# jwliao1209/DiffMusic

Hardware: AMD Instinct MI355X
Metric: denoising steps/sec (10 s clip, 200-step DPS) (higher is better)
Workload: dtype f16; 1 GPU; MusicLDM + DPS music_inpainting, 10 s @16 kHz, 200-step schedule, batch 8 per GPU (BASELINE.json configs[1]); global_batch=8, clips_per_gpu=8, lanes=1, parallelism=clip-sharded x1 (RCCL world size 1, no per-step collective), finite=True, nan_steps=0, settle_steps=10, cached_reference_transform=True, launched_by=single process

## Files before the change

### diffmusic_amd/_lib.py

```python
import ctypes as C
import os

_HERE = os.path.dirname(os.path.abspath(__file__))
LIB_PATH = os.environ.get("DMX_LIB_PATH") or os.path.join(_HERE, "lib", "libdiffmusic_hip.so")
MAX_STAGES = 8


class HifiGanConfig(C.Structure):
    _fields_ = [("model_in_dim", C.c_int), ("upsample_initial_channel", C.c_int), ("num_upsamples", C.c_int),
                ("upsample_rates", C.c_int * MAX_STAGES), ("upsample_kernel_sizes", C.c_int * MAX_STAGES),
                ("num_kernels", C.c_int), ("resblock_kernel_sizes", C.c_int * MAX_STAGES),
                ("num_dilations", C.c_int), ("resblock_dilation_sizes", C.c_int * (MAX_STAGES * MAX_STAGES)),
                ("leaky_relu_slope", C.c_float)]


class VaeConfig(C.Structure):
    _fields_ = [("latent_channels", C.c_int), ("out_channels", C.c_int), ("num_blocks", C.c_int),
                ("block_out_channels", C.c_int * MAX_STAGES), ("layers_per_block", C.c_int),
                ("norm_num_groups", C.c_int), ("eps", C.c_float)]


class UNetConfig(C.Structure):
    _fields_ = [("in_channels", C.c_int), ("out_channels", C.c_int), ("num_blocks", C.c_int),
                ("block_out_channels", C.c_int * MAX_STAGES), ("layers_per_block", C.c_int),
# ... 1 lines not shown
                ("down_attn", C.c_int * MAX_STAGES), ("up_attn", C.c_int * MAX_STAGES),
                ("class_embed_dim", C.c_int), ("num_attn_per_layer", C.c_int), ("attn_cross_dims", C.c_int * 4)]


class HtsatConfig(C.Structure):
    _fields_ = [("spec_size", C.c_int), ("num_mel_bins", C.c_int), ("patch_size", C.c_int), ("embed_dim", C.c_int), ("window_size", C.c_int),
                ("num_stages", C.c_int), ("depths", C.c_int * 4), ("num_heads", C.c_int * 4), ("ln_eps", C.c_float), ("bn_eps", C.c_float)]


class GemmDesc(C.Structure):
    _fields_ = [("A", C.c_void_p), ("W", C.c_void_p), ("C", C.c_void_p), ("C2", C.c_void_p),
                ("bias", C.c_void_p), ("rowbias", C.c_void_p), ("R", C.c_void_p), ("X", C.c_void_p),
                ("M", C.c_int), ("N", C.c_int), ("K", C.c_int), ("ldw", C.c_int),
                ("Hi", C.c_int), ("Wi", C.c_int), ("Ci", C.c_int), ("lda", C.c_int),
                ("Hq", C.c_int), ("Wq", C.c_int), ("sy", C.c_int), ("sx", C.c_int),
                ("ntaps", C.c_int),
                ("Ho", C.c_int), ("Wo", C.c_int), ("ldc", C.c_int), ("osy", C.c_int), ("ooy", C.c_int),
                ("osx", C.c_int), ("oox", C.c_int),
                ("ldr", C.c_int), ("ldx", C.c_int), ("ldc2", C.c_int),
                ("Z", C.c_int), ("Zi", C.c_int),
                ("sAo", C.c_longlong), ("sAi", C.c_longlong), ("sWo", C.c_longlong), ("sWi", C.c_longlong),
                ("sCo", C.c_longlong), ("sCi", C.c_longlong),
                ("alpha", C.c_float), ("act_slope", C.c_float), ("mask_slope", C.c_float),
                ("flags", C.c_int),
                ("tdy", C.c_byte * 16), ("tdx", C.c_byte * 16), ("resid_inv_slope", C.c_float), ("tile_cfg", C.c_int), ("ldrb", C.c_int), ("ksplit", C.c_int),
                ("XB", C.c_void_p), ("B2", C.c_void_p), ("ldxb", C.c_int), ("ldb2", C.c_int),
                ("colsum", C.c_void_p), ("ln_eps", C.c_float), ("rowstats_in", C.c_void_p), ("rowstats_out", C.c_void_p), ("nslots", C.c_int),
                ("gn_part", C.c_void_p), ("gnb_x", C.c_void_p), ("gnb_scale", C.c_void_p), ("gnb_shift", C.c_void_p),
                ("gnb_ldx", C.c_int), ("gnb_silu", C.c_int), ("gnb_stats", C.c_void_p), ("gnb_cpg", C.c_int)]


EPI_BIAS, EPI_ROWBIAS, EPI_RESID, EPI_ACCUM, EPI_MASK, EPI_LRELU2, EPI_TANH, EPI_F32OUT, EPI_NO_C, EPI_RESID_INV, EPI_MASKBITS, EPI_BITS2, EPI_SOFTBWD = \
    1, 2, 4, 8, 16, 32, 64, 128, 256, 512, 1024, 2048, 4096
EPI_GEGLU, EPI_LNFOLD, EPI_ROWSTATS, EPI_GNSTATS, EPI_GNBWD = 8192, 16384, 32768, 65536, 131072

_SIGS = {
    "dmx_abi_version": (C.c_int, []),
    "dmx_act_dtype": (C.c_int, []),
    "dmx_last_error": (C.c_char_p, []),
    "dmx_hifigan_create": (C.c_void_p, [C.POINTER(HifiGanConfig)]),
    "dmx_vae_decoder_create": (C.c_void_p, [C.POINTER(VaeConfig)]),
    "dmx_unet_create": (C.c_void_p, [C.POINTER(UNetConfig)]),
    "dmx_model_destroy": (None, [C.c_void_p]),
    "dmx_model_num_params": (C.c_int, [C.c_void_p]),
    "dmx_model_param_name": (C.c_char_p, [C.c_void_p, C.c_int]),
    "dmx_model_param_numel": (C.c_size_t, [C.c_void_p, C.c_int]),
    "dmx_model_param_ndim": (C.c_int, [C.c_void_p, C.c_int]),
    "dmx_model_param_dim": (C.c_int, [C.c_void_p, C.c_int, C.c_int]),
    "dmx_model_load_param": (C.c_int, [C.c_void_p, C.c_char_p, C.c_void_p, C.c_size_t]),
    "dmx_model_finalize": (C.c_int, [C.c_void_p, C.c_void_p]),
    "dmx_hifigan_out_len": (C.c_int, [C.c_void_p, C.c_int]),
    "dmx_hifigan_workspace_bytes": (C.c_size_t, [C.c_void_p, C.c_int, C.c_int]),
    "dmx_hifigan_fwd": (C.c_int, [C.c_void_p, C.c_void_p, C.c_void_p, C.c_int, C.c_int, C.c_void_p, C.c_size_t, C.c_void_p]),
    "dmx_hifigan_bwd": (C.c_int, [C.c_void_p, C.c_void_p, C.c_void_p, C.c_void_p]),
    "dmx_hifigan_fwd_dead": (C.c_int, [C.c_void_p, C.c_void_p, C.c_void_p, C.c_int, C.c_int, C.c_int, C.c_int, C.c_void_p, C.c_size_t,
                                       C.c_void_p]),
    "dmx_hifigan_dead_plan": (C.c_int, [C.c_void_p, C.POINTER(C.c_int), C.POINTER(C.c_int), C.POINTER(C.c_int), C.POINTER(C.c_int), C.c_int]),
    "dmx_conv_dead_rows": (C.c_int, [C.c_int] * 9 + [C.POINTER(C.c_int), C.POINTER(C.c_int)]),
    "dmx_vae_workspace_bytes": (C.c_size_t, [C.c_void_p, C.c_int, C.c_int, C.c_int]),
    "dmx_vae_decode_fwd": (C.c_int, [C.c_void_p, C.c_void_p, C.c_float, C.c_void_p, C.c_void_p, C.c_int, C.c_int, C.c_int,
                                     C.c_int, C.c_void_p, C.c_size_t, C.c_void_p]),
    "dmx_vae_decode_bwd": (C.c_int, [C.c_void_p, C.c_void_p, C.c_float, C.c_void_p, C.c_void_p]),
    "dmx_vae_encoder_create": (C.c_void_p, [C.POINTER(VaeConfig)]),
    "dmx_vae_encoder_workspace_bytes": (C.c_size_t, [C.c_void_p, C.c_int, C.c_int, C.c_int]),
    "dmx_vae_encode_fwd": (C.c_int, [C.c_void_p, C.c_void_p, C.c_float, C.c_void_p, C.c_int, C.c_int, C.c_int, C.c_void_p, C.c_size_t,
                                     C.c_void_p]),
    "dmx_latent_init": (C.c_int, [C.c_void_p] * 6 + [C.c_int] * 3 + [C.c_float] * 3 + [C.c_void_p]),
    "dmx_conv2d_raw": (C.c_int, [C.c_void_p] * 4 + [C.c_int] * 9 + [C.c_void_p]),
    "dmx_unet_workspace_bytes": (C.c_size_t, [C.c_void_p, C.c_int, C.c_int, C.c_int]),
    "dmx_unet_fwd": (C.c_int, [C.c_void_p, C.c_void_p, C.c_void_p, C.c_void_p, C.c_void_p, C.c_int, C.c_int, C.c_int,
                               C.c_void_p, C.c_size_t, C.c_void_p]),
    "dmx_unet_fwd_ctx": (C.c_int, [C.c_void_p] * 5 + [C.c_int, C.c_void_p, C.c_int, C.c_void_p, C.c_void_p, C.c_int, C.c_int, C.c_int,
                                   C.c_void_p, C.c_size_t, C.c_void_p]),
    "dmx_unet_workspace_bytes_ctx": (C.c_size_t, [C.c_void_p, C.c_int, C.c_int, C.c_int, C.c_int, C.c_int]),
    "dmx_htsat_create": (C.c_void_p, [C.POINTER(HtsatConfig)]),
    "dmx_htsat_feature_dims": (C.c_int, [C.c_void_p, C.POINTER(C.c_int), C.POINTER(C.c_int)]),
    "dmx_htsat_workspace_bytes": (C.c_size_t, [C.c_void_p, C.c_int, C.c_int]),
    "dmx_htsat_fwd": (C.c_int, [C.c_void_p, C.c_void_p, C.c_int, C.c_int, C.c_void_p, C.c_int, C.c_void_p, C.c_size_t, C.c_void_p]),
    "dmx_htsat_bwd": (C.c_int, [C.c_void_p, C.c_void_p, C.c_void_p, C.c_void_p, C.c_void_p]),
    "dmx_htsat_tape_raw": (C.c_size_t, [C.c_void_p, C.c_int, C.c_int, C.c_int, C.c_void_p, C.c_size_t, C.c_void_p]),
    "dmx_gram_fwd": (C.c_int, [C.c_void_p, C.c_void_p, C.c_int, C.c_int, C.c_int, C.c_void_p]),
    "dmx_gram_bwd": (C.c_int, [C.c_void_p, C.c_void_p, C.c_void_p, C.c_int, C.c_int, C.c_int, C.c_void_p]),
    "dmx_gemm_raw": (C.c_int, [C.c_void_p, C.c_size_t, C.c_void_p]),
    "dmx_prof_begin": (None, []),
    "dmx_prof_end": (C.c_int, [C.POINTER(C.c_double), C.POINTER(C.c_double)]),
    "dmx_flash_attn_raw": (C.c_int, [C.c_void_p, C.c_void_p, C.c_void_p, C.c_void_p, C.c_void_p] + [C.c_int] * 6 + [C.c_float, C.c_void_p]),
    "dmx_flash_attn_ld_raw": (C.c_int, [C.c_void_p] * 5 + [C.c_int] * 8 + [C.c_float, C.POINTER(C.c_int), C.c_void_p]),
    "dmx_softmax_raw": (C.c_int, [C.c_void_p] * 3 + [C.c_longlong, C.c_int, C.c_longlong, C.c_longlong, C.c_int, C.c_void_p]),
    "dmx_softmax_act_raw": (C.c_int, [C.c_void_p] * 3 + [C.c_longlong, C.c_int, C.c_longlong, C.c_int, C.c_void_p]),
    "dmx_transpose_raw": (C.c_int, [C.c_void_p, C.c_void_p, C.c_int, C.c_int, C.c_longlong, C.c_longlong, C.c_int, C.c_int] + [C.c_longlong] * 4
                          + [C.c_void_p]),
    "dmx_rowdot_raw": (C.c_int, [C.c_void_p] * 3 + [C.c_longlong, C.c_int, C.c_longlong, C.c_longlong, C.c_void_p]),
    "dmx_layernorm_raw": (C.c_int, [C.c_void_p] * 4 + [C.c_int, C.c_int, C.c_float, C.c_void_p]),
    "dmx_geglu_raw": (C.c_int, [C.c_void_p, C.c_void_p, C.c_longlong, C.c_int, C.c_void_p]),
    "dmx_gemm_splitk_workspace": (C.c_int, [C.c_void_p, C.c_size_t]),
    "dmx_conv_pair_raw": (C.c_int, [C.c_void_p, C.c_void_p, C.c_size_t, C.c_void_p]),
    "dmx_conv_pair_group_raw": (C.c_int, [C.c_int, C.c_void_p, C.c_void_p, C.c_size_t, C.c_void_p]),
    "dmx_conv_pair_dead_raw": (C.c_int, [C.c_void_p, C.c_void_p, C.c_size_t, C.POINTER(C.c_int), C.POINTER(C.c_int), C.POINTER(C.c_int), C.c_void_p]),
    "dmx_conv_pair_group_dead_raw": (C.c_int, [C.c_int, C.c_void_p, C.c_void_p, C.c_size_t, C.POINTER(C.c_int), C.c_void_p]),
    "dmx_groupnorm_scratch_floats": (C.c_size_t, [C.c_int, C.c_int, C.c_int]),
    "dmx_groupnorm_raw": (C.c_int, [C.c_void_p] * 8 + [C.c_int] * 4 + [C.c_float, C.c_int, C.c_void_p]),
    "dmx_groupnorm_part_floats": (C.c_size_t, [C.c_int, C.c_int, C.c_int]),
    "dmx_groupnorm_parts_raw": (C.c_int, [C.c_void_p] * 7 + [C.c_int] * 4 + [C.c_float, C.c_int, C.c_int, C.c_void_p, C.c_void_p, C.c_void_p]),
    "dmx_gemm_last_tile_rows_raw": (C.c_int, []),
    "dmx_groupnorm_bwd_raw": (C.c_int, [C.c_void_p] * 10 + [C.c_int] * 6 + [C.c_void_p, C.c_void_p, C.c_void_p]),
    "dmx_prof_dominant": (C.c_int, [C.POINTER(C.c_double)] * 3),
    "dmx_audio_create": (C.c_void_p, [C.c_int, C.c_int, C.c_int, C.c_int, C.c_void_p]),
    "dmx_audio_destroy": (None, [C.c_void_p]),
    "dmx_audio_num_frames": (C.c_int, [C.c_void_p, C.c_int]),
    "dmx_audio_num_bins": (C.c_int, [C.c_void_p]),
    "dmx_audio_state_bytes": (C.c_size_t, [C.c_void_p, C.c_int, C.c_int]),
    "dmx_audio_transform_fwd": (C.c_int, [C.c_void_p, C.c_void_p, C.c_longlong, C.c_void_p, C.c_void_p, C.c_int, C.c_int, C.c_int,
                                          C.c_int, C.c_float, C.c_float, C.c_void_p]),
    "dmx_audio_transform_bwd": (C.c_int, [C.c_void_p, C.c_void_p, C.c_void_p, C.c_longlong, C.c_void_p, C.c_int, C.c_int, C.c_int,
                                          C.c_int, C.c_float, C.c_float, C.c_int, C.c_void_p]),
    "dmx_audio_is_fused": (C.c_int, [C.c_void_p, C.c_int]),
    "dmx_audio_guidance_fwd": (C.c_int, [C.c_void_p, C.c_void_p, C.c_longlong, C.c_void_p, C.c_void_p, C.c_longlong, C.c_void_p, C.c_void_p,
                                         C.c_int, C.c_int, C.c_int, C.c_int, C.c_float, C.c_float, C.c_void_p]),
    "dmx_audio_guidance_bwd": (C.c_int, [C.c_void_p, C.c_void_p, C.c_longlong, C.c_void_p, C.c_void_p, C.c_longlong, C.c_float, C.c_void_p,
                                         C.c_void_p, C.c_longlong, C.c_int, C.c_void_p, C.c_int, C.c_int, C.c_int, C.c_int, C.c_float, C.c_float,
                                         C.c_void_p]),
    "dmx_audio_guidance_fwd_ex": (C.c_int, [C.c_void_p, C.c_void_p, C.c_longlong, C.c_void_p, C.c_void_p, C.c_longlong, C.c_void_p, C.c_void_p,
                                            C.c_int, C.c_int, C.c_int, C.c_int, C.c_float, C.c_float, C.c_void_p, C.c_longlong, C.c_void_p,
                                            C.c_float, C.c_void_p]),
    "dmx_audio_guidance_bwd_ex": (C.c_int, [C.c_void_p, C.c_void_p, C.c_longlong, C.c_void_p, C.c_void_p, C.c_longlong, C.c_float, C.c_void_p,
                                            C.c_void_p, C.c_longlong, C.c_int, C.c_void_p, C.c_int, C.c_int, C.c_int, C.c_int, C.c_float, C.c_float,
                                            C.c_void_p, C.c_longlong, C.c_void_p, C.c_float, C.c_void_p]),
    "dmx_audio_guidance_fwd_shaped": (C.c_int, [C.c_void_p, C.c_void_p, C.c_longlong, C.c_void_p, C.c_void_p, C.c_longlong, C.c_void_p, C.c_void_p,
                                                C.c_int, C.c_int, C.c_int, C.c_int, C.c_float, C.c_float, C.c_void_p, C.c_longlong, C.c_void_p,
                                                C.c_float, C.c_void_p, C.c_void_p]),
    "dmx_audio_guidance_bwd_shaped": (C.c_int, [C.c_void_p, C.c_void_p, C.c_longlong, C.c_void_p, C.c_void_p, C.c_longlong, C.c_float, C.c_void_p,
                                                C.c_void_p, C.c_longlong, C.c_int, C.c_void_p, C.c_int, C.c_int, C.c_int, C.c_int, C.c_float, C.c_float,
                                                C.c_void_p, C.c_longlong, C.c_void_p, C.c_float, C.c_void_p, C.c_void_p]),
    "dmx_clip_fwd": (C.c_int, [C.c_void_p, C.c_longlong, C.c_void_p, C.c_void_p, C.c_longlong, C.c_int, C.c_int, C.c_void_p]),
    "dmx_clip_bwd": (C.c_int, [C.c_void_p, C.c_longlong, C.c_void_p, C.c_longlong, C.c_void_p, C.c_void_p, C.c_longlong, C.c_int, C.c_int, C.c_int,
                               C.c_void_p]),
    "dmx_declip_project": (C.c_int, [C.c_void_p, C.c_longlong, C.c_void_p, C.c_longlong, C.c_void_p, C.c_void_p, C.c_longlong, C.c_int, C.c_int,
                                     C.c_void_p]),
    "dmx_drc_fwd": (C.c_int, [C.c_void_p, C.c_longlong, C.c_void_p, C.c_longlong, C.c_void_p, C.c_void_p, C.c_int, C.c_int] + [C.c_float] * 6 +
                    [C.c_void_p]),
    "dmx_drc_bwd": (C.c_int, [C.c_void_p, C.c_longlong, C.c_void_p, C.c_longlong, C.c_void_p, C.c_void_p, C.c_void_p, C.c_void_p, C.c_longlong,
                              C.c_int, C.c_int, C.c_int] + [C.c_float] * 6 + [C.c_void_p]),
    "dmx_drc_fwd_p": (C.c_int, [C.c_void_p, C.c_longlong, C.c_void_p, C.c_longlong, C.c_void_p, C.c_void_p, C.c_void_p, C.c_int, C.c_int, C.c_float,
                                C.c_void_p]),
    "dmx_drc_bwd_p": (C.c_int, [C.c_void_p, C.c_longlong, C.c_void_p, C.c_longlong] + [C.c_void_p] * 6 + [C.c_longlong, C.c_int, C.c_int, C.c_int,
                                                                                                        C.c_float, C.c_void_p]),
    "dmx_drc_pgrad": (C.c_int, [C.c_void_p] * 6 + [C.c_int, C.c_int, C.c_float, C.c_void_p]),
    "dmx_drc_update": (C.c_int, [C.c_void_p] * 5 + [C.c_int] * 3 + [C.c_void_p] + [C.c_double] * 3 + [C.c_float, C.c_void_p, C.c_void_p, C.c_void_p]),
    "dmx_warp_fwd": (C.c_int, [C.c_void_p, C.c_longlong, C.c_void_p, C.c_longlong, C.c_void_p, C.c_int, C.c_int, C.c_void_p]),
    "dmx_warp_bwd": (C.c_int, [C.c_void_p, C.c_void_p, C.c_longlong, C.c_void_p, C.c_int, C.c_int, C.c_int, C.c_void_p]),
    "dmx_warp_wgrad": (C.c_int, [C.c_void_p, C.c_void_p, C.c_longlong, C.c_void_p, C.c_longlong, C.c_void_p, C.c_int, C.c_int, C.c_void_p]),
    "dmx_warp_update": (C.c_int, [C.c_void_p] * 5 + [C.c_int] * 4 + [C.c_double] * 5 + [C.c_int, C.c_void_p]),
    "dmx_click_detect": (C.c_int, [C.c_void_p, C.c_longlong] + [C.c_void_p] * 5 + [C.c_int, C.c_int, C.c_float, C.c_float, C.c_void_p]),
    "dmx_click_mask": (C.c_int, [C.c_void_p, C.c_void_p, C.c_void_p, C.c_int, C.c_int, C.c_int, C.c_void_p]),
    "dmx_mask_rows": (C.c_int, [C.c_void_p, C.c_longlong, C.c_void_p, C.c_longlong, C.c_void_p, C.c_int, C.c_int, C.c_int, C.c_void_p]),
    "dmx_declick_blend": (C.c_int, [C.c_void_p, C.c_longlong, C.c_void_p, C.c_longlong, C.c_void_p, C.c_longlong, C.c_void_p, C.c_int, C.c_int,
                                    C.c_int, C.c_void_p]),
    "dmx_noise_add": (C.c_int, [C.c_void_p, C.c_void_p, C.c_void_p, C.c_longlong, C.c_float, C.c_void_p]),
    "dmx_audio_stft_mag": (C.c_int, [C.c_void_p, C.c_void_p, C.c_longlong, C.c_void_p, C.c_void_p, C.c_int, C.c_int, C.c_void_p]),
    "dmx_audio_stft_mag_bwd": (C.c_int, [C.c_void_p, C.c_void_p, C.c_void_p, C.c_longlong, C.c_void_p, C.c_int, C.c_int, C.c_int, C.c_void_p]),
    "dmx_audio_tf_frames": (C.c_int, [C.c_int]),
    "dmx_audio_tf_gain": (C.c_int, [C.c_void_p, C.c_void_p, C.c_longlong, C.c_void_p, C.c_longlong, C.c_void_p, C.c_longlong, C.c_int, C.c_int, C.c_int,
                                    C.c_void_p]),
    "dmx_audio_tf_curve": (C.c_int, [C.c_void_p, C.c_void_p, C.c_longlong, C.c_void_p, C.c_longlong, C.c_void_p, C.c_longlong, C.c_int, C.c_int, C.c_int,
                                     C.c_void_p]),
    "dmx_audio_tf_wgrad_segments": (C.c_int, [C.c_int]),
    "dmx_audio_tf_wgrad": (C.c_int, [C.c_void_p, C.c_void_p, C.c_longlong, C.c_void_p, C.c_longlong, C.c_void_p, C.c_int, C.c_int, C.c_void_p]),
    "dmx_audio_eq_update": (C.c_int, [C.c_void_p, C.c_int] + [C.c_void_p] * 3 + [C.c_int, C.c_int] + [C.c_double] * 4 + [C.c_int, C.c_void_p]),
    "dmx_audio_melscale": (C.c_int, [C.c_void_p, C.c_void_p, C.c_void_p, C.c_int, C.c_int, C.c_float, C.c_float, C.c_void_p]),
    "dmx_mask_apply": (C.c_int, [C.c_void_p, C.c_longlong, C.c_void_p, C.c_void_p, C.c_longlong, C.c_int, C.c_int, C.c_int, C.c_void_p]),
    "dmx_l2_loss": (C.c_int, [C.c_void_p, C.c_longlong, C.c_void_p, C.c_void_p, C.c_void_p, C.c_int, C.c_longlong, C.c_float, C.c_void_p]),
    "dmx_track_stitch_fwd": (C.c_int, [C.c_void_p, C.c_longlong, C.c_void_p, C.POINTER(C.c_int)] + [C.c_int] * 4 + [C.c_void_p]),
    "dmx_track_stitch_bwd": (C.c_int, [C.c_void_p, C.c_void_p, C.c_longlong, C.POINTER(C.c_int)] + [C.c_int] * 5 + [C.c_void_p]),
    "dmx_stem_mix_fwd": (C.c_int, [C.c_void_p, C.c_longlong, C.c_void_p, C.POINTER(C.c_float)] + [C.c_int] * 3 + [C.c_void_p]),
    "dmx_stem_mix_bwd": (C.c_int, [C.c_void_p, C.c_void_p, C.c_longlong, C.POINTER(C.c_float)] + [C.c_int] * 4 + [C.c_void_p]),
    "dmx_stem_project": (C.c_int, [C.c_void_p, C.c_longlong, C.c_void_p, C.c_void_p, C.POINTER(C.c_float), C.c_int, C.c_int, C.c_void_p]),
    "dmx_grad_normalize": (C.c_int, [C.c_void_p, C.c_void_p, C.c_int, C.c_longlong, C.c_float, C.c_void_p]),
    "dmx_fir_fwd": (C.c_int, [C.c_void_p, C.c_longlong, C.c_void_p, C.c_void_p, C.c_longlong] + [C.c_int] * 7 + [C.c_void_p]),
    "dmx_fir_bwd": (C.c_int, [C.c_void_p, C.c_longlong, C.c_void_p, C.c_void_p, C.c_void_p, C.c_longlong] + [C.c_int] * 7 + [C.c_void_p]),
    "dmx_fir_clip_fwd": (C.c_int, [C.c_void_p, C.c_longlong, C.c_void_p, C.c_void_p, C.c_longlong] + [C.c_int] * 4 + [C.c_void_p]),
    "dmx_fir_clip_bwd": (C.c_int, [C.c_void_p, C.c_longlong, C.c_void_p, C.c_void_p, C.c_void_p, C.c_longlong] + [C.c_int] * 4 + [C.c_void_p]),
    "dmx_fir_wgrad_workspace_floats": (C.c_size_t, [C.c_int, C.c_int, C.c_int]),
    "dmx_fir_wgrad": (C.c_int, [C.c_void_p, C.c_longlong, C.c_void_p, C.c_longlong, C.c_void_p, C.c_size_t] + [C.c_int] * 4 + [C.c_void_p]),
    "dmx_ir_update": (C.c_int, [C.c_void_p, C.c_int] + [C.c_void_p] * 4 + [C.c_int, C.c_int] + [C.c_double] * 4 + [C.c_int, C.c_void_p]),
    "dmx_sched_pred_x0": (C.c_int, [C.c_void_p, C.c_void_p, C.c_void_p, C.c_longlong, C.c_float, C.c_void_p]),
    "dmx_sched_pred_x0_ex": (C.c_int, [C.c_void_p, C.c_void_p, C.c_void_p, C.c_longlong, C.c_float, C.c_int, C.c_float, C.c_void_p]),
    "dmx_sched_step_ex": (C.c_int, [C.c_int] + [C.c_void_p] * 9 + [C.c_int, C.c_int] + [C.c_float] * 5 + [C.c_int, C.c_int, C.c_float, C.c_void_p]),
    "dmx_sched_cfg_combine": (C.c_int, [C.c_void_p, C.c_void_p, C.c_longlong, C.c_float, C.c_void_p]),
    "dmx_randn_philox": (C.c_int, [C.c_void_p, C.c_int, C.c_longlong, C.POINTER(C.c_ulonglong), C.c_ulonglong, C.c_void_p]),
    "dmx_sched_step": (C.c_int, [C.c_int] + [C.c_void_p] * 9 + [C.c_int, C.c_int] + [C.c_float] * 5 + [C.c_int, C.c_void_p]),
}

ADDED_IN_V4 = ("dmx_vae_encoder_create", "dmx_vae_encoder_workspace_bytes", "dmx_vae_encode_fwd", "dmx_latent_init",
               "dmx_track_stitch_fwd", "dmx_track_stitch_bwd", "dmx_audio_guidance_fwd_shaped", "dmx_audio_guidance_bwd_shaped",
               "dmx_clip_fwd", "dmx_clip_bwd", "dmx_declip_project", "dmx_hifigan_fwd_dead", "dmx_hifigan_dead_plan", "dmx_conv_dead_rows",
               "dmx_fir_clip_fwd", "dmx_fir_clip_bwd", "dmx_fir_wgrad", "dmx_fir_wgrad_workspace_floats", "dmx_ir_update",
               "dmx_stem_mix_fwd", "dmx_stem_mix_bwd", "dmx_stem_project", "dmx_audio_tf_gain", "dmx_audio_tf_frames",
               "dmx_audio_tf_curve", "dmx_audio_tf_wgrad_segments", "dmx_audio_tf_wgrad", "dmx_audio_eq_update", "dmx_drc_fwd", "dmx_drc_bwd",
               "dmx_warp_fwd", "dmx_warp_bwd", "dmx_warp_wgrad", "dmx_warp_update", "dmx_drc_fwd_p", "dmx_drc_bwd_p", "dmx_drc_pgrad",
               "dmx_drc_update", "dmx_click_detect", "dmx_click_mask", "dmx_mask_rows", "dmx_declick_blend")

_lib = None


def check_symbols(h, path=LIB_PATH):
    for name in ADDED_IN_V4:
        if not hasattr(h, name):
            raise RuntimeError(f"{path} reports ABI version {ABI_VERSION} but does not export `{name}` (a build from before the VAE "
                               "encoder / track-mode / declipping / blind-dereverberation / source-separation / time-frequency-masking / blind-equalisation / de-compression / wow-and-flutter / blind-wow-and-flutter / blind-de-compression / declicking entry points): rebuild it (python -m diffmusic_amd.build --force)")


def lib():
    global _lib
    if _lib is None:
        if not os.path.exists(LIB_PATH):
            raise RuntimeError(f"{LIB_PATH} is missing: build it with `python -m diffmusic_amd.build` "
                               "(the diffmusic_amd hot path has no CPU fallback)")
        h = C.CDLL(LIB_PATH)
        for name, (res, args) in _SIGS.items():
            if not hasattr(h, name):
                continue
            fn = getattr(h, name)
            fn.restype, fn.argtypes = res, args
        if h.dmx_abi_version() != ABI_VERSION:
            raise RuntimeError(f"libdiffmusic_hip.so ABI version {h.dmx_abi_version()} != {ABI_VERSION} expected by this package: rebuild it "
                               "(python -m diffmusic_amd.build --force)")
        check_symbols(h)
        _lib = h
    return _lib


ABI_VERSION = 4


def act_dtype():
    import torch
    return torch.float16 if lib().dmx_act_dtype() == 1 else torch.bfloat16


class DmxError(RuntimeError):
    pass


def check(rc, what=""):
    if rc != 0:
        msg = lib().dmx_last_error()
        raise DmxError(f"{what} failed with code {rc}: {msg.decode() if msg else ''}")
```

### diffmusic_amd/csrc/capi.hip

```cpp
#include "conv_pair.h"
#include "models.h"

#define M_IMPL(m) ((m) ? (m)->impl : nullptr)
#define ST(s) ((hipStream_t)(s))

extern "C" {

int dmx_abi_version(void) { return DMX_ABI_VERSION; }
int dmx_act_dtype(void) { return DMX_ACT_DTYPE; }

dmx_model* dmx_hifigan_create(const dmx_hifigan_config* cfg) {
  if (!cfg || cfg->num_upsamples > DMX_MAX_STAGES || cfg->num_kernels > DMX_MAX_STAGES || cfg->num_dilations > DMX_MAX_STAGES) {
    dmx_set_error("bad hifigan config");
    return nullptr;
  }
  return new dmx_model{dmx_make_hifigan(cfg)};
}
dmx_model* dmx_vae_decoder_create(const dmx_vae_config* cfg) {
  if (!cfg || cfg->num_blocks > DMX_MAX_STAGES) { dmx_set_error("bad vae config"); return nullptr; }
  Model* m = dmx_make_vae(cfg);
  return m ? new dmx_model{m} : nullptr;
}
dmx_model* dmx_unet_create(const dmx_unet_config* cfg) {
  if (!cfg || cfg->num_blocks > DMX_MAX_STAGES) { dmx_set_error("bad unet config"); return nullptr; }
// ... 81 lines not shown
  return dmx_vae_enc_ws_impl(m->impl, batch, frames, bins);
}
int dmx_vae_encode_fwd(dmx_model* m, const float* mel, float log_floor, float* moments, int batch, int frames, int bins, void* ws,
                       size_t ws_bytes, void* stream) {
  int rc = check(m, DMX_MODEL_VAE_ENC);
  if (rc) return rc;
  if (!ws) { dmx_set_error("null workspace"); return DMX_ERR_WORKSPACE; }
  return dmx_vae_enc_fwd_impl(m->impl, mel, log_floor, moments, batch, frames, bins, ws, ws_bytes, ST(stream));
}
int dmx_latent_init(const float* moments, float* mean, float* logvar, float* x, const float* eps, const float* noise, int batch,
                    int latent_channels, int hw, float sqrt_abar, float scaling_factor, float sqrt_1m_abar, void* stream) {
  return dmx_latent_init_impl(moments, mean, logvar, x, eps, noise, batch, latent_channels, hw, sqrt_abar, scaling_factor, sqrt_1m_abar, ST(stream));
}
int dmx_conv2d_raw(const float* w_host, const float* b_host, const void* x, void* y, int B, int Hi, int Wi, int Ci, int Co, int k, int stride,
                   int pad_lo, int pad_hi, void* stream) {
  return dmx_conv2d_raw_impl(w_host, b_host, (const act_t*)x, (act_t*)y, B, Hi, Wi, Ci, Co, k, stride, pad_lo, pad_hi, ST(stream));
}

dmx_model* dmx_htsat_create(const dmx_htsat_config* cfg) {
  Model* impl = dmx_make_htsat(cfg);
  if (!impl) return nullptr;
  return new dmx_model{impl};
}
int dmx_htsat_feature_dims(dmx_model* m, int* tokens, int* channels) {
  if (!m || !m->impl || m->impl->kind != DMX_MODEL_HTSAT) { dmx_set_error("wrong model handle"); return DMX_ERR_STATE; }
  dmx_htsat_dims_impl(m->impl, tokens, channels);
  return DMX_OK;
}
size_t dmx_htsat_workspace_bytes(dmx_model* m, int batch, int frames) {
  if (!m || !m->impl || m->impl->kind != DMX_MODEL_HTSAT) return 0;
  return dmx_htsat_ws_impl(m->impl, batch, frames);
}
int dmx_htsat_fwd(dmx_model* m, const float* mel, int batch, int frames, float* feat, int keep_state, void* ws, size_t ws_bytes, void* stream) {
  int rc = check(m, DMX_MODEL_HTSAT);
  if (rc) return rc;
  if (!ws) { dmx_set_error("null workspace"); return DMX_ERR_WORKSPACE; }
  return dmx_htsat_fwd_impl(m->impl, mel, batch, frames, feat, keep_state, ws, ws_bytes, ST(stream));
}
int dmx_htsat_bwd(dmx_model* m, const float* dfeat, const float* scale, float* dmel, void* stream) {
  int rc = check(m, DMX_MODEL_HTSAT);
  if (rc) return rc;
  return dmx_htsat_bwd_impl(m->impl, dfeat, scale, dmel, ST(stream));
}
size_t dmx_htsat_tape_raw(dmx_model* m, int stage, int block, int which, void* dst, size_t dst_elems, void* stream) {
  if (!m || !m->impl || m->impl->kind != DMX_MODEL_HTSAT) return 0;
  const act_t* p = nullptr;
  const size_t n = dmx_htsat_tape_impl(m->impl, stage, block, which, &p);
  if (n && dst && dst_elems >= n) (void)hipMemcpyAsync(dst, p, n * sizeof(act_t), hipMemcpyDeviceToDevice, ST(stream));
  return n;
}
int dmx_gram_fwd(const float* F, float* G, int batch, int tokens, int channels, void* stream) {
  const int rc = dmx_gram_fwd_impl(F, G, batch, tokens, channels, ST(stream));
  if (rc == DMX_ERR_SHAPE) dmx_set_error("gram: 1 <= tokens <= 96");
  return rc;
}
int dmx_gram_bwd(const float* F, const float* dG, float* dF, int batch, int tokens, int channels, void* stream) {
  return dmx_gram_bwd_impl(F, dG, dF, batch, tokens, channels, ST(stream));
}

size_t dmx_unet_workspace_bytes(dmx_model* m, int batch, int h, int w) { return dmx_unet_ws_impl(m->impl, batch, h, w, 0, 0); }
size_t dmx_unet_workspace_bytes_ctx(dmx_model* m, int batch, int h, int w, int n0, int n1) { return dmx_unet_ws_impl(m->impl, batch, h, w, n0, n1); }
int dmx_unet_fwd(dmx_model* m, const float* x, const float* t, const float* class_labels, float* eps, int batch, int h, int w,
                 void* ws, size_t ws_bytes, void* stream) {
  int rc = check(m, DMX_MODEL_UNET);
  if (rc) return rc;
  if (!ws) { dmx_set_error("null workspace"); return DMX_ERR_WORKSPACE; }
  return dmx_unet_fwd_impl(m->impl, x, t, class_labels, eps, batch, h, w, ws, ws_bytes, ST(stream), nullptr, 0, nullptr, 0, nullptr);
}
int dmx_unet_fwd_ctx(dmx_model* m, const float* x, const float* t, const float* class_labels, const float* ctx0, int n0,
                     const float* ctx1, int n1, const float* bias1, float* eps, int batch, int h, int w, void* ws, size_t ws_bytes,
                     void* stream) {
  int rc = check(m, DMX_MODEL_UNET);
  if (rc) return rc;
  if (!ws) { dmx_set_error("null workspace"); return DMX_ERR_WORKSPACE; }
  return dmx_unet_fwd_impl(m->impl, x, t, class_labels, eps, batch, h, w, ws, ws_bytes, ST(stream), ctx0, n0, ctx1, n1, bias1);
}

static thread_local int g_raw_gn_rows = 0;
int dmx_gemm_raw(const void* desc, size_t desc_bytes, void* stream) {
  if (desc_bytes != sizeof(GemmDesc)) { dmx_set_error("GemmDesc size mismatch: %zu vs %zu", desc_bytes, sizeof(GemmDesc)); return DMX_ERR_SHAPE; }
  return dmx_gemm_launch(*reinterpret_cast<const GemmDesc*>(desc), ST(stream), &g_raw_gn_rows);
}
int dmx_gemm_last_tile_rows_raw(void) { return g_raw_gn_rows; }

int dmx_conv_pair_raw(const void* desc_a, const void* desc_b, size_t desc_bytes, void* stream) {
  if (desc_bytes != sizeof(GemmDesc)) { dmx_set_error("GemmDesc size mismatch: %zu vs %zu", desc_bytes, sizeof(GemmDesc)); return DMX_ERR_SHAPE; }
  const GemmDesc* a = reinterpret_cast<const GemmDesc*>(desc_a);
  const GemmDesc& b = *reinterpret_cast<const GemmDesc*>(desc_b);
  if (!dmx_conv_pair_eligible(a, b)) { dmx_set_error("shape not handled by the fused convolution-pair kernel"); return DMX_ERR_SHAPE; }
  return dmx_conv_pair_launch(a, b, ST(stream));
}

int dmx_conv_pair_group_raw(int n, const void* descs_a, const void* descs_b, size_t desc_bytes, void* stream) {
  if (desc_bytes != sizeof(GemmDesc)) { dmx_set_error("GemmDesc size mismatch: %zu vs %zu", desc_bytes, sizeof(GemmDesc)); return DMX_ERR_SHAPE; }
  if (n < 1 || n > 3) { dmx_set_error("conv pair group: 1..3 problems"); return DMX_ERR_SHAPE; }
  const GemmDesc* a = reinterpret_cast<const GemmDesc*>(descs_a);
  const GemmDesc* b = reinterpret_cast<const GemmDesc*>(descs_b);
  const GemmDesc* pa[3]; const GemmDesc* pb[3];
  for (int j = 0; j < n; ++j) { pa[j] = a + j; pb[j] = b + j; }
  const int rc = dmx_conv_pair_group_launch(n, pa, pb, ST(stream));
  if (rc == DMX_ERR_SHAPE) dmx_set_error("shape not handled by the fused convolution-pair kernel");
  return rc;
}

static PairDead pair_dead_of(const int* d) { PairDead pd; pd.skip0 = d[0]; pd.skip1 = d[1]; pd.zero0 = d[2]; pd.zero1 = d[3]; return pd; }

int dmx_conv_pair_dead_raw(const void* desc_a, const void* desc_b, size_t desc_bytes, const int* dead, int* skipped, int* total, void* stream) {
  if (skipped) *skipped = 0;
  if (total) *total = 0;
  if (desc_bytes != sizeof(GemmDesc)) { dmx_set_error("GemmDesc size mismatch: %zu vs %zu", desc_bytes, sizeof(GemmDesc)); return DMX_ERR_SHAPE; }
  const GemmDesc* a = reinterpret_cast<const GemmDesc*>(desc_a);
  const GemmDesc& b = *reinterpret_cast<const GemmDesc*>(desc_b);
  if (!dmx_conv_pair_eligible(a, b)) { dmx_set_error("shape not handled by the fused convolution-pair kernel"); return DMX_ERR_SHAPE; }
  PairDead pd;
  if (dead) pd = pair_dead_of(dead);
  int sk = 0, tot = 0;
  dmx_conv_pair_slabs(a, b, dead ? &pd : nullptr, &sk, &tot);
  if (skipped) *skipped = sk;
  if (total) *total = tot;
  const int rc = dmx_conv_pair_launch(a, b, ST(stream), dead ? &pd : nullptr);
  if (rc == DMX_ERR_SHAPE) dmx_set_error("dead rows not handled by the fused convolution-pair kernel (zero rows need the residual to be stage a's input)");
  return rc;
}

int dmx_conv_pair_group_dead_raw(int n, const void* descs_a, const void* descs_b, size_t desc_bytes, const int* dead, void* stream) {
  if (desc_bytes != sizeof(GemmDesc)) { dmx_set_error("GemmDesc size mismatch: %zu vs %zu", desc_bytes, sizeof(GemmDesc)); return DMX_ERR_SHAPE; }
  if (n < 1 || n > 3) { dmx_set_error("conv pair group: 1..3 problems"); return DMX_ERR_SHAPE; }
  const GemmDesc* a = reinterpret_cast<const GemmDesc*>(descs_a);
  const GemmDesc* b = reinterpret_cast<const GemmDesc*>(descs_b);
  const GemmDesc* pa[3]; const GemmDesc* pb[3];
  PairDead pd[3];
  for (int j = 0; j < n; ++j) { pa[j] = a + j; pb[j] = b + j; if (dead) pd[j] = pair_dead_of(dead + 4 * j); }
  const int rc = dmx_conv_pair_group_launch(n, pa, pb, ST(stream), dead ? pd : nullptr);
  if (rc == DMX_ERR_SHAPE) dmx_set_error("shape not handled by the fused convolution-pair kernel");
  return rc;
}

int dmx_flash_attn_raw(const void* q, const void* k, const void* v, void* o, const float* colbias, int B, int Nq, int Nk, int ldv, int C,
                       int heads, float scale, void* stream) {
  const int rc = dmx_flash_attn_fwd((const act_t*)q, (const act_t*)k, (const act_t*)v, (act_t*)o, colbias, B, Nq, Nk, C, heads, scale,
                                    ST(stream), 0, 0, ldv);
  if (rc == DMX_ERR_SHAPE) dmx_set_error("flash attention: unsupported head_dim / strides");
  return rc;
}

int dmx_flash_attn_ld_raw(const void* q, const void* k, const void* v, void* o, const float* colbias, int B, int Nq, int Nk, int ldq, int ldk,
                          int ldv, int C, int heads, float scale, int* qt_out, void* stream) {
  if (qt_out) *qt_out = 0;
  if (B < 1 || heads < 1 || C < heads || C % heads) { dmx_set_error("flash attention: C %d is not heads %d x head_dim", C, heads); return DMX_ERR_SHAPE; }
  const int rc = dmx_flash_attn_fwd((const act_t*)q, (const act_t*)k, (const act_t*)v, (act_t*)o, colbias, B, Nq, Nk, C, heads, scale,
                                    ST(stream), ldq, ldk, ldv, qt_out);
  if (rc == DMX_ERR_SHAPE)
    dmx_set_error("flash attention: head_dim %d (multiples of 8 up to 96), Nq %d, Nk %d (>= 1) or row strides %d / %d / %d (multiples of 8) unsupported",
                  C / heads, Nq, Nk, ldq, ldk, ldv);
  return rc;
}

int dmx_softmax_raw(const float* S, void* P, const float* colbias, long long rows, int N, long long lds, long long ldp, int rows_per_bias,
                    void* stream) {
  const int rc = dmx_softmax_fwd(S, (act_t*)P, colbias, rows, N, lds, ldp, rows_per_bias, ST(stream));
  if (rc == DMX_ERR_SHAPE) dmx_set_error("softmax: N %d (a multiple of 4, <= 4096), lds %lld, ldp %lld (multiples of 4) unsupported", N, lds, ldp);
  return rc;
}
int dmx_softmax_act_raw(const void* S, void* P, const float* colbias, long long rows, int N, long long ldp, int rows_per_bias, void* stream) {
  const int rc = dmx_softmax_act((const act_t*)S, (act_t*)P, colbias, rows, N, ldp, rows_per_bias, ST(stream));
  if (rc == DMX_ERR_SHAPE) dmx_set_error("softmax: N %d (a multiple of 4, <= 4096), ldp %lld (a multiple of 4) unsupported", N, ldp);
// ... 75 lines not shown
```

### diffmusic_amd/csrc/dmx_common.h

```cpp
#pragma once
#include <hip/hip_runtime.h>
#include <stdint.h>
#include <stddef.h>

typedef uint16_t act_t;

#define DMX_OK 0
#define DMX_ERR_SHAPE (-1)
#define DMX_ERR_WORKSPACE (-2)
#define DMX_ERR_PARAM (-3)
#define DMX_ERR_STATE (-4)
#define DMX_ERR_LAUNCH (-5)

typedef __attribute__((ext_vector_type(4))) float f32x4;
#ifdef DMX_BF16
typedef __bf16 native16_t;
typedef __attribute__((ext_vector_type(8))) __bf16 frag8_t;
#define DMX_MFMA16(a, b, c) __builtin_amdgcn_mfma_f32_16x16x32_bf16(a, b, c, 0, 0, 0)
#define DMX_ACT_DTYPE 0
#else
typedef _Float16 native16_t;
typedef __attribute__((ext_vector_type(8))) _Float16 frag8_t;
#define DMX_MFMA16(a, b, c) __builtin_amdgcn_mfma_f32_16x16x32_f16(a, b, c, 0, 0, 0)
#define DMX_ACT_DTYPE 1
// ... 33 lines not shown
  float r = 0.f;
  for (int i = 0; i < nw; ++i) r += sh[i];
  return r;
}
__device__ __forceinline__ float block_max(float v, float* sh) {
  v = wave_max(v);
  const int w = threadIdx.x >> 6, nw = blockDim.x >> 6;
  __syncthreads();
  if ((threadIdx.x & 63) == 0) sh[w] = v;
  __syncthreads();
  float r = -3.0e38f;
  for (int i = 0; i < nw; ++i) r = fmaxf(r, sh[i]);
  return r;
}

static inline int cdiv(int a, int b) { return (a + b - 1) / b; }
static inline size_t align_up(size_t v, size_t a) { return (v + a - 1) / a * a; }

#define DMX_MAX_TAPS 16
enum {
  EPI_BIAS = 1,
  EPI_ROWBIAS = 2,
  EPI_RESID = 4,
  EPI_ACCUM = 8,
  EPI_MASK = 16,
  EPI_LRELU2 = 32,
  EPI_TANH = 64,
  EPI_F32OUT = 128,
  EPI_NO_C = 256,
  EPI_RESID_INV = 512,
  EPI_MASKBITS = 1024,
  EPI_BITS2 = 2048,
  EPI_GEGLU = 8192,
  EPI_LNFOLD = 16384,
  EPI_ROWSTATS = 32768,
  EPI_GNSTATS = 65536,
  EPI_GNBWD = 131072,
  EPI_BIASINIT = 262144,
  EPI_SOFTBWD = 4096
};

struct GemmDesc {
  const act_t* A;
  const act_t* W;
  void* C;
  act_t* C2;
  const float* bias;
  const float* rowbias;
  const act_t* R;
  const act_t* X;
  int M, N, K;
  int ldw;
  int Hi, Wi, Ci, lda;
  int Hq, Wq, sy, sx;
  int ntaps;
  int Ho, Wo, ldc, osy, ooy, osx, oox;
  int ldr, ldx, ldc2;
  int Z, Zi;
  long long sAo, sAi, sWo, sWi, sCo, sCi;
  float alpha, act_slope, mask_slope;
  int flags;
  signed char tdy[DMX_MAX_TAPS], tdx[DMX_MAX_TAPS];
  float resid_inv_slope;
  int tile_cfg;
  int ldrb;
  int ksplit;
  const unsigned char* XB;
  unsigned char* B2;
  int ldxb, ldb2;
  const float* colsum;
  float ln_eps;
  const float* rowstats_in;
  float* rowstats_out;
  int nslots;
  float* gn_part;
  const act_t* gnb_x;
  const float* gnb_scale;
  const float* gnb_shift;
  int gnb_ldx, gnb_silu;
  const float* gnb_stats;
  int gnb_cpg;
};

int dmx_gemm_launch(const GemmDesc& d, hipStream_t stream, int* gn_rows = nullptr);
void dmx_gemm_set_splitk_workspace(float* ws, size_t bytes);
void dmx_gemm_release_splitk_workspace(const float* ws);
int dmx_gemm_launch_ln(int cfg, const GemmDesc& d, hipStream_t stream);
int dmx_gemm_launch_rowstats(int cfg, const GemmDesc& d, hipStream_t stream);
int dmx_gemm_launch_gnstats(int cfg, const GemmDesc& d, hipStream_t stream, int* gn_rows);
bool dmx_prof_is_active();
```

### diffmusic_amd/csrc/gemm_conv.hip

```cpp
#include "gemm_tile.h"

namespace {
template <int BM, int BN, int WM, int WN, int NSTAGE>
int launch_glds(const GemmDesc& d, hipStream_t stream) {
  if (d.flags & EPI_SOFTBWD) {
    if constexpr (BM == 256 && BN == 256) return launch_glds_t<BM, BN, WM, WN, NSTAGE, 2>(d, stream);
    else return DMX_ERR_SHAPE;
  }
  if (d.flags & EPI_GEGLU) return launch_glds_t<BM, BN, WM, WN, NSTAGE, 3>(d, stream);
  return (d.flags & (EPI_MASKBITS | EPI_BITS2)) ? launch_glds_t<BM, BN, WM, WN, NSTAGE, 1>(d, stream)
                                                : launch_glds_t<BM, BN, WM, WN, NSTAGE, 0>(d, stream);
}

template <int BM, int BN, int WM, int WN>
int launch_cfg(const GemmDesc& d, hipStream_t stream) {
  if (d.flags & EPI_SOFTBWD) return DMX_ERR_SHAPE;
  if (d.flags & EPI_GEGLU) {
    if constexpr ((BN / WN) % 32 == 0) return launch_cfg_t<BM, BN, WM, WN, 3>(d, stream);
    else return DMX_ERR_SHAPE;
  }
  return (d.flags & (EPI_MASKBITS | EPI_BITS2)) ? launch_cfg_t<BM, BN, WM, WN, 1>(d, stream) : launch_cfg_t<BM, BN, WM, WN, 0>(d, stream);
}

}
// ... 180 lines not shown
  }
  if (flags & EPI_RESID) {
    const uint2 rr = *reinterpret_cast<const uint2*>(p.R + row * p.ldr + n);
    const float is = (flags & EPI_RESID_INV) ? p.resid_inv_slope : 1.f;
    const float x[4] = {alo(rr.x), ahi(rr.x), alo(rr.y), ahi(rr.y)};
#pragma unroll
    for (int e = 0; e < 4; ++e) a[e] += fminf(x[e], x[e] * is);
  }
#pragma unroll
  for (int e = 0; e < 4; ++e) a[e] *= p.alpha;
  if (!(flags & EPI_NO_C))
    *reinterpret_cast<uint2*>(reinterpret_cast<act_t*>(p.C) + row * p.ldc + n) = make_uint2(pack2a(a[0], a[1]), pack2a(a[2], a[3]));
  if (flags & EPI_LRELU2) {
    const float sl = p.act_slope;
    *reinterpret_cast<uint2*>(p.C2 + row * p.ldc2 + n) =
        make_uint2(pack2a(fmaxf(a[0], a[0] * sl), fmaxf(a[1], a[1] * sl)), pack2a(fmaxf(a[2], a[2] * sl), fmaxf(a[3], a[3] * sl)));
  }
}

int splitk_plan(const GemmDesc& d, int* tile) {
  static const bool off = getenv("DMX_NO_SPLITK") != nullptr;
  if (off || !g_splitk_ws || d.Z != 1 || !glds_ok(d)) return 1;
  if (d.flags & (EPI_ACCUM | EPI_F32OUT | EPI_TANH | EPI_MASKBITS | EPI_BITS2 | EPI_SOFTBWD | EPI_GEGLU | EPI_LNFOLD | EPI_ROWSTATS)) return 1;
  if (!(d.osy == 1 && d.osx == 1 && d.ooy == 0 && d.oox == 0 && d.Ho == d.Hq && d.Wo == d.Wq)) return 1;
  if ((d.N & 7) || (d.ldc & 3)) return 1;
  const int nk = (d.K + BK - 1) / BK;
  auto fits = [&](int ks) { return ks >= 2 && ks <= nk && (size_t)ks * d.M * d.N * sizeof(float) <= g_splitk_bytes; };
  auto dma_tile = [](int t) { return t == 1 || t == 2 || (t >= 7 && t <= 19); };
  if (d.tile_cfg >= 100) { *tile = d.tile_cfg % 100; return fits(d.tile_cfg / 100) && dma_tile(*tile) ? d.tile_cfg / 100 : 1; }
  if (d.tile_cfg) return 1;
  for (const TileEntry* e = g_tile_table; e->cfg; ++e)
    if (e->M == d.M && e->N == d.N && e->K == d.K && e->Z == d.Z) {
      if (e->cfg < 100) return 1;
      *tile = e->cfg % 100;
      return fits(e->cfg / 100) && dma_tile(*tile) ? e->cfg / 100 : 1;
    }
  if (d.M > 8192) return 1;
  const long long tiles = (long long)cdiv(d.M, 64) * cdiv(d.N, 64);
  if (nk < 24 || tiles >= 256) return 1;
  int ks = (int)(1024 / tiles);
  if (ks > nk / 8) ks = nk / 8;
  if (ks > 8) ks = 8;
  while (ks > 1 && !fits(ks)) --ks;
  *tile = d.N % 128 == 0 && d.M >= 4096 ? 14 : 12;
  return ks < 2 ? 1 : ks;
}

int launch_splitk(const GemmDesc& d, int ks, int tile, hipStream_t stream) {
  GemmDesc g = d;
  g.ksplit = ks;
  g.flags = EPI_F32OUT;
  g.C = g_splitk_ws; g.C2 = nullptr; g.ldc = d.N; g.alpha = 1.f;
  g.bias = nullptr; g.rowbias = nullptr; g.R = nullptr; g.X = nullptr;
  g.Ho = d.Hq; g.Wo = d.Wq;
  g.tile_cfg = 0;
  int rc = launch_by_cfg(tile, g, stream);
  if (rc != DMX_OK) return rc;
  const long long nthr = (long long)d.M * (d.N >> 2);
  hipLaunchKernelGGL(splitk_epilogue_kernel, dim3((unsigned)((nthr + 255) / 256)), dim3(256), 0, stream, d, g_splitk_ws, ks);
  g_last_cfg = 100 * ks + tile;
  return hipGetLastError() == hipSuccess ? DMX_OK : DMX_ERR_LAUNCH;
}
}

void dmx_gemm_set_splitk_workspace(float* ws, size_t bytes) { g_splitk_ws = ws; g_splitk_bytes = bytes; }
void dmx_gemm_release_splitk_workspace(const float* ws) { if (g_splitk_ws == ws) { g_splitk_ws = nullptr; g_splitk_bytes = 0; } }

int dmx_prof_open(hipStream_t st) {
  if (!g_prof) return -1;
  ProfRec r;
  memset(&r, 0, sizeof(r));
  (void)hipEventCreate(&r.a); (void)hipEventCreate(&r.b);
  (void)hipEventRecord(r.a, st);
  g_prof_recs.push_back(r);
  return (int)g_prof_recs.size() - 1;
}
void dmx_prof_close(int rec, hipStream_t st, double flops, double bytes, int M, int N, int K, int taps, int flags, int cfg) {
  if (rec < 0 || rec >= (int)g_prof_recs.size()) return;
  ProfRec& r = g_prof_recs[rec];
  (void)hipEventRecord(r.b, st);
  r.flops = flops; r.bytes = bytes; r.M = M; r.N = N; r.K = K; r.Z = 1; r.taps = taps; r.flags = flags; r.cfg = cfg;
}

int dmx_gemm_launch(const GemmDesc& d, hipStream_t stream, int* gn_rows) {
  if (gn_rows) *gn_rows = 0;
  if (d.M <= 0 || d.N <= 0 || d.K <= 0) return DMX_ERR_SHAPE;
  if ((d.Ci & 7) || (d.N & 3) || (d.K & 7) || (d.lda & 7) || (d.ldw & 7) || (d.ldc & 3)) return DMX_ERR_SHAPE;
  if (d.ntaps < 1 || d.ntaps > DMX_MAX_TAPS || d.K != d.ntaps * d.Ci) return DMX_ERR_SHAPE;
  if (d.Z < 1 || d.Zi < 1) return DMX_ERR_SHAPE;
  if ((d.flags & EPI_LRELU2) && !(d.act_slope >= 0.f && d.act_slope <= 1.f)) return DMX_ERR_SHAPE;
  if ((d.flags & EPI_RESID_INV) && !(d.resid_inv_slope >= 1.f)) return DMX_ERR_SHAPE;
  if (d.flags & EPI_SOFTBWD) {
    if ((d.flags & ~(EPI_SOFTBWD)) || ((d.N | d.ldc | d.ldx) & 7) || !d.X || !d.rowbias || d.Zi != 1 || d.ntaps != 1) return DMX_ERR_SHAPE;
    if (!(d.osy == 1 && d.osx == 1 && d.ooy == 0 && d.oox == 0 && d.Ho == d.Hq && d.Wo == d.Wq)) return DMX_ERR_SHAPE;
  }
  if (d.flags & EPI_GEGLU) {
    if ((d.flags & ~(EPI_GEGLU | EPI_BIAS | EPI_LNFOLD)) || (d.N & 31) || (d.ldc & 7) || d.ldc < d.N / 2 || d.alpha != 1.f) return DMX_ERR_SHAPE;
    if ((d.ldr | d.ldx | d.ldc2) & 7) return DMX_ERR_SHAPE;
    if (!(d.osy == 1 && d.osx == 1 && d.ooy == 0 && d.oox == 0 && d.Ho == d.Hq && d.Wo == d.Wq)) return DMX_ERR_SHAPE;
  }
  if (d.flags & (EPI_MASKBITS | EPI_BITS2)) {
    if ((d.flags & EPI_F32OUT) || ((d.N | d.ldc | d.ldr | d.ldx | d.ldc2) & 7) || d.Z != 1) return DMX_ERR_SHAPE;
    if ((d.flags & EPI_MASKBITS) && (!d.XB || d.ldxb * 8 < d.N)) return DMX_ERR_SHAPE;
    if ((d.flags & EPI_BITS2) && (!d.B2 || d.ldb2 * 8 < d.N)) return DMX_ERR_SHAPE;
  }
  if ((d.flags & EPI_LNFOLD) && (d.flags & EPI_BIAS)) {
    GemmDesc q = d;
    q.flags &= ~EPI_BIAS;
    return dmx_gemm_launch(q, stream, gn_rows);
  }
  if (d.flags & EPI_LNFOLD) {
    if (d.ntaps != 1 || d.K != d.Ci || !d.colsum || !d.rowstats_in || d.nslots < 1 || d.Z != 1 ||
        (d.flags & (EPI_F32OUT | EPI_MASK | EPI_MASKBITS | EPI_BITS2 | EPI_SOFTBWD | EPI_ACCUM | EPI_TANH | EPI_LRELU2 | EPI_ROWSTATS)))
      return DMX_ERR_SHAPE;
  }
  if (d.flags & EPI_ROWSTATS) {
    if (!d.rowstats_out || d.nslots * 32 != d.N || d.Z != 1 || ((d.ldc | d.ldr) & 7) ||
        (d.flags & (EPI_F32OUT | EPI_MASK | EPI_MASKBITS | EPI_BITS2 | EPI_SOFTBWD | EPI_ACCUM | EPI_TANH | EPI_LRELU2 | EPI_GEGLU | EPI_NO_C)))
      return DMX_ERR_SHAPE;
    if (!(d.osy == 1 && d.osx == 1 && d.ooy == 0 && d.oox == 0 && d.Ho == d.Hq && d.Wo == d.Wq)) return DMX_ERR_SHAPE;
  }
  if (d.flags & (EPI_GNSTATS | EPI_GNBWD)) {
    bool can = d.gn_part && d.Z == 1 && !(d.flags & (EPI_F32OUT | EPI_NO_C | EPI_GEGLU | EPI_SOFTBWD | EPI_MASKBITS | EPI_BITS2 | EPI_LNFOLD | EPI_ROWSTATS | EPI_LRELU2)) &&
               !((d.N | d.ldc | d.ldr | d.ldx | d.ldc2) & 7) && (d.flags & (EPI_GNSTATS | EPI_GNBWD)) != (EPI_GNSTATS | EPI_GNBWD);
    if (d.flags & EPI_GNBWD) can = can && d.gnb_x && d.gnb_scale && d.gnb_shift && d.gnb_stats && !(d.gnb_ldx & 7) && d.gnb_cpg >= 4 && !(d.gnb_cpg & 3) && d.N % d.gnb_cpg == 0;
    int kt = 12;
    if (!can || splitk_plan(d, &kt) > 1) { GemmDesc q = d; q.flags &= ~(EPI_GNSTATS | EPI_GNBWD); return dmx_gemm_launch(q, stream, gn_rows); }
  }
  int ktile = 12;
  const int ksp = splitk_plan(d, &ktile);
  if (ksp <= 1 && d.tile_cfg >= 100) return DMX_ERR_SHAPE;
  if (!g_prof) return ksp > 1 ? launch_splitk(d, ksp, ktile, stream) : launch_dispatch(d, stream, gn_rows);
  ProfRec r;
  (void)hipEventCreate(&r.a); (void)hipEventCreate(&r.b);
  r.flops = 2.0 * d.M * (double)d.N * d.K * d.Z;
  {
    const double mn = (double)d.M * d.N * d.Z;
    double by = 2.0 * d.M * (double)d.Ci * d.Z + 2.0 * d.N * (double)d.K * (d.sWo ? d.Z : 1);
    if (!(d.flags & EPI_NO_C)) by += mn * ((d.flags & EPI_F32OUT) ? 4.0 : 2.0);
    if (d.flags & EPI_ACCUM) by += mn * ((d.flags & EPI_F32OUT) ? 4.0 : 2.0);
    if (d.flags & (EPI_RESID | EPI_RESID_INV)) by += mn * 2.0;
    if (d.flags & (EPI_MASK | EPI_SOFTBWD)) by += mn * 2.0;
    if (d.flags & EPI_MASKBITS) by += mn / 8.0;
    if (d.flags & EPI_BITS2) by += mn / 8.0;
    if (d.C2 && (d.flags & EPI_LRELU2)) by += mn * 2.0;
    r.bytes = by;
  }
  r.M = d.M; r.N = d.N; r.K = d.K; r.Z = d.Z; r.taps = d.ntaps; r.flags = d.flags;
  (void)hipEventRecord(r.a, stream);
  const int rc = ksp > 1 ? launch_splitk(d, ksp, ktile, stream) : launch_dispatch(d, stream, gn_rows);
  (void)hipEventRecord(r.b, stream);
  r.cfg = g_last_cfg;
  g_prof_recs.push_back(r);
  return rc;
}
```

### diffmusic_amd/csrc/gemm_tile.h

```cpp
#pragma once
#include "dmx_common.h"
#include <type_traits>
#include <cstdlib>

#include "gemm_epilogue.h"
#include "conv_pair.h"

namespace {

constexpr int BK = 64;
constexpr int DMX_DEF_BIG = 0;

template <int BM, int BN, int NT>
__device__ __forceinline__ void ln_prologue(const GemmDesc& p, int m0, int n0, float2* s_ln, float* s_cs) {
  constexpr int TPR = NT / BM >= 4 ? 4 : (NT / BM >= 2 ? 2 : 1);
  const int tid = threadIdx.x, ns = p.nslots;
  const int r = tid / TPR, sub = tid - r * TPR;
  const float inv_c = 1.f / (float)p.K;
  if (r < BM) {
    const int m = m0 + r;
    const bool row_ok = m < p.M;
    const float2* rs = reinterpret_cast<const float2*>(p.rowstats_in) + (long long)(row_ok ? m : 0) * ns;
    float si = 0.f, qi = 0.f;
    for (int t0 = 0; t0 < ns; t0 += TPR * 8) {
      float2 v[8];
#pragma unroll
      for (int u = 0; u < 8; ++u) {
        const int t = t0 + u * TPR + sub;
        v[u] = (row_ok && t < ns) ? rs[t] : make_float2(0.f, 0.f);
      }
#pragma unroll
      for (int u = 0; u < 8; ++u) { si += v[u].x; qi += v[u].y; }
    }
    if constexpr (TPR >= 2) { si += __shfl_xor(si, 1, 64); qi += __shfl_xor(qi, 1, 64); }
    if constexpr (TPR >= 4) { si += __shfl_xor(si, 2, 64); qi += __shfl_xor(qi, 2, 64); }
    const float mean = si * inv_c;
    if (sub == 0) s_ln[r] = make_float2(mean, rsqrtf(fmaxf(qi * inv_c - mean * mean, 0.f) + p.ln_eps));
  }
  for (int c = tid; c < BN; c += NT) {
    const bool ok = n0 + c < p.N;
    s_cs[c] = ok ? p.colsum[n0 + c] : 0.f;
    s_cs[BN + c] = (ok && p.bias) ? p.bias[n0 + c] : 0.f;
  }
}
template <int FM, int FN, int BN>
__device__ __forceinline__ void ln_apply(f32x4 (&acc)[FM][FN], const float2* s_ln, const float* s_cs, int r0, int c0, int lr, int lq) {
#pragma unroll
  for (int j = 0; j < FN; ++j) {
    const float4 cs = *reinterpret_cast<const float4*>(s_cs + c0 + j * 16 + lq * 4);
    const float4 bs = *reinterpret_cast<const float4*>(s_cs + BN + c0 + j * 16 + lq * 4);
#pragma unroll
    for (int i = 0; i < FM; ++i) {
      const float2 st = s_ln[r0 + i * 16 + lr];
      const float mean = st.x, rstd = st.y;
      f32x4& a = acc[i][j];
      a[0] = __builtin_fmaf(rstd, a[0] - mean * cs.x, bs.x); a[1] = __builtin_fmaf(rstd, a[1] - mean * cs.y, bs.y);
      a[2] = __builtin_fmaf(rstd, a[2] - mean * cs.z, bs.z); a[3] = __builtin_fmaf(rstd, a[3] - mean * cs.w, bs.w);
    }
  }
}

template <int BM, int BN, int WM, int WN, int EM, bool LNF = false>
__global__ __launch_bounds__(WM* WN * 64) void gemm_kernel(const GemmDesc p) {
  constexpr int NT = WM * WN * 64;
  constexpr int TM = BM / WM, TN = BN / WN;
  constexpr int FM = TM / 16, FN = TN / 16;
  constexpr int A_PER = BM * 8 / NT, B_PER = BN * 8 / NT;
  constexpr int ROWS_PER_PASS = NT / 8;
  constexpr int A_BYTES = BM * 128, B_BYTES = BN * 128, STAGE = A_BYTES + B_BYTES;
  static_assert(A_PER >= 1 && B_PER >= 1, "tile too small for the thread count");

  extern __shared__ __attribute__((aligned(16))) char smem[];
  short2* s_taps = reinterpret_cast<short2*>(smem + 2 * STAGE);

  const int tid = threadIdx.x;
  const int tiles_n = (p.N + BN - 1) / BN;
  const int tn = blockIdx.x % tiles_n, tm = blockIdx.x / tiles_n;
  const int z = blockIdx.y;
  const int zo = z / p.Zi, zi = z - zo * p.Zi;
  const act_t* __restrict__ Ab = p.A + zo * p.sAo + zi * p.sAi;
  const act_t* __restrict__ Wb = p.W + zo * p.sWo + zi * p.sWi;
  const long long coff = zo * p.sCo + zi * p.sCi;

  if (tid < DMX_MAX_TAPS) s_taps[tid] = make_short2(p.tdy[tid], p.tdx[tid]);
  float2* s_ln = reinterpret_cast<float2*>(smem + 2 * STAGE + DMX_MAX_TAPS * 4);
  float* s_cs = reinterpret_cast<float*>(smem + 2 * STAGE + DMX_MAX_TAPS * 4 + BM * 8);
  int m0t = tm * BM, mlim = p.M;
  if constexpr (EM == 5 || EM == 6) {
    const int P = p.Hq * p.Wq;
    if (P % TM != 0) {
      const int tpi = (P + BM - 1) / BM, b = tm / tpi;
      m0t = b * P + (tm - b * tpi) * BM;
      mlim = (b + 1) * P;
    }
  }
  if constexpr (LNF) ln_prologue<BM, BN, NT>(p, m0t, tn * BN, s_ln, s_cs);

  const int cc = tid & 7, r0 = tid >> 3;
  const int cpt = p.Ci >> 3;
  const int HqWq = p.Hq * p.Wq;
  const act_t* a_base[A_PER];
  int a_iy[A_PER], a_ix[A_PER];
#pragma unroll
  for (int i = 0; i < A_PER; ++i) {
    const int m = m0t + r0 + i * ROWS_PER_PASS;
    if (m < mlim) {
      const int b = m / HqWq, rem = m - b * HqWq;
      const int qy = rem / p.Wq, qx = rem - qy * p.Wq;
      a_base[i] = Ab + (long long)b * p.Hi * p.Wi * p.lda;
      a_iy[i] = qy * p.sy;
      a_ix[i] = qx * p.sx;
    } else {
      a_base[i] = Ab;
      a_iy[i] = -(1 << 20);
      a_ix[i] = 0;
    }
  }
  const act_t* w_base[B_PER];
  bool w_ok[B_PER];
#pragma unroll
  for (int i = 0; i < B_PER; ++i) {
    const int n = tn * BN + r0 + i * ROWS_PER_PASS;
    w_ok[i] = n < p.N;
    w_base[i] = Wb + (long long)(w_ok[i] ? n : 0) * p.ldw;
  }
  __syncthreads();

  uint4 ra[A_PER], rb[B_PER];
  const int kchunks = p.K >> 3;
  auto load_tile = [&](int ks) {
    const int kc = ks * 8 + cc;
    const int tap = kc / cpt;
    const int cin = (kc - tap * cpt) << 3;
    const bool kval = kc < kchunks;
    const short2 t = s_taps[tap & (DMX_MAX_TAPS - 1)];
#pragma unroll
    for (int i = 0; i < A_PER; ++i) {
      const int iy = a_iy[i] + t.x, ix = a_ix[i] + t.y;
      const bool ok = kval && (unsigned)iy < (unsigned)p.Hi && (unsigned)ix < (unsigned)p.Wi;
      ra[i] = make_uint4(0, 0, 0, 0);
      if (ok) ra[i] = *reinterpret_cast<const uint4*>(a_base[i] + (long long)(iy * p.Wi + ix) * p.lda + cin);
    }
#pragma unroll
    for (int i = 0; i < B_PER; ++i) {
      rb[i] = make_uint4(0, 0, 0, 0);
      if (kval && w_ok[i]) rb[i] = *reinterpret_cast<const uint4*>(w_base[i] + (kc << 3));
    }
  };
  auto store_tile = [&](int buf) {
    char* sa = smem + buf * STAGE;
    char* sb = sa + A_BYTES;
#pragma unroll
    for (int i = 0; i < A_PER; ++i) {
      const int r = r0 + i * ROWS_PER_PASS;
      *reinterpret_cast<uint4*>(sa + r * 128 + ((cc ^ (r & 7)) << 4)) = ra[i];
    }
#pragma unroll
    for (int i = 0; i < B_PER; ++i) {
      const int r = r0 + i * ROWS_PER_PASS;
      *reinterpret_cast<uint4*>(sb + r * 128 + ((cc ^ (r & 7)) << 4)) = rb[i];
    }
  };

  const int wave = tid >> 6, lane = tid & 63;
  const int wm = wave / WN, wn = wave - wm * WN;
  const int lr = lane & 15, lq = lane >> 4;

  f32x4 acc[FM][FN];
  if (p.flags & EPI_BIASINIT) {
#pragma unroll
    for (int j = 0; j < FN; ++j) {
      const int n = tn * BN + wn * TN + j * 16 + lq * 4;
      float bb[4];
#pragma unroll
      for (int e = 0; e < 4; ++e) bb[e] = n + e < p.N ? p.bias[n + e] : 0.f;
#pragma unroll
      for (int i = 0; i < FM; ++i) acc[i][j] = f32x4{bb[0], bb[1], bb[2], bb[3]};
    }
  } else {
#pragma unroll
    for (int i = 0; i < FM; ++i)
#pragma unroll
      for (int j = 0; j < FN; ++j) acc[i][j] = f32x4{0.f, 0.f, 0.f, 0.f};
  }

  const int nk = (p.K + BK - 1) / BK;
  load_tile(0);
  store_tile(0);
  __syncthreads();

  for (int ks = 0; ks < nk; ++ks) {
    const int cur = ks & 1;
    if (ks + 1 < nk) load_tile(ks + 1);
    const char* sa = smem + cur * STAGE + (wm * TM + lr) * 128;
    const char* sb = smem + cur * STAGE + A_BYTES + (wn * TN + lr) * 128;
#pragma unroll
    for (int kk = 0; kk < 2; ++kk) {
      const int sw = ((kk * 4 + lq) ^ (lr & 7)) << 4;
      frag8_t af[FM], wf[FN];
#pragma unroll
      for (int i = 0; i < FM; ++i) af[i] = *reinterpret_cast<const frag8_t*>(sa + i * 16 * 128 + sw);
#pragma unroll
      for (int j = 0; j < FN; ++j) wf[j] = *reinterpret_cast<const frag8_t*>(sb + j * 16 * 128 + sw);
#pragma unroll
      for (int i = 0; i < FM; ++i)
#pragma unroll
        for (int j = 0; j < FN; ++j)
          acc[i][j] = DMX_MFMA16(wf[j], af[i], acc[i][j]);
    }
    if (ks + 1 < nk) store_tile(cur ^ 1);
    __syncthreads();
  }
  if constexpr (LNF) ln_apply<FM, FN, BN>(acc, s_ln, s_cs, wm * TM, wn * TN, lr, lq);

  if ((p.flags & EPI_F32OUT) || ((p.N | p.ldc | p.ldr | p.ldx | p.ldc2) & 7)) {
    gemm_epilogue<FM, FN>(p, acc, m0t + wm * TM, tn * BN + wn * TN, lr, lq, coff, HqWq);
  } else {
    constexpr int EPI_CH = EpiChunk<FM>::CH;
    constexpr int EPI_WAVE_BYTES = EPI_CH * (FN * 32 + 16) + EPI_CH * 12;
    static_assert(EPI_WAVE_BYTES * WM * WN <= 2 * (BM + BN) * 128, "epilogue staging does not fit the stage buffers");
    gemm_epilogue_lds<FM, FN, EM>(p, acc, m0t + wm * TM, tn * BN + wn * TN, lane, coff, HqWq, smem + wave * EPI_WAVE_BYTES, mlim);
  }
}

constexpr unsigned OOB = 0x80000000u;

#ifdef DMX_GEMM_STAMPS
__device__ unsigned long long g_gemm_stamps[8192 * 6];
#define DMX_GSTAMP(i) do { gstamp_v[i] = wall_clock64(); } while (0)
#else
#define DMX_GSTAMP(i) do { } while (0)
#endif

template <int BM, int BN, int WM, int WN, int NSTAGE, int EM, bool LNF = false>
__device__ __forceinline__ void glds_tile(const GemmDesc& p, char* smem, const int m0, const int tn, const int mlim) {
  constexpr int NW = WM * WN;
  constexpr int TM = BM / WM, TN = BN / WN;
  constexpr int FM = TM / 16, FN = TN / 16;
  constexpr int A_ISS = BM / 8 / NW, B_ISS = BN / 8 / NW;
  constexpr int A_BYTES = BM * 128, B_BYTES = BN * 128, STAGE = A_BYTES + B_BYTES;
  static_assert(A_ISS >= 1 && B_ISS >= 1, "tile too small");

  constexpr int PER = A_ISS + B_ISS;
  constexpr int KEEP = (NSTAGE - 2) * PER;

  const int tid = threadIdx.x;
  const int wave = __builtin_amdgcn_readfirstlane(tid >> 6), lane = tid & 63;
#ifdef DMX_GEMM_STAMPS
  unsigned long long gstamp_v[5] = {0, 0, 0, 0, 0};
#endif
  DMX_GSTAMP(0);
  const int z = blockIdx.y;
  const int zo = z / p.Zi, zi = z - zo * p.Zi;
  const act_t* Ab = p.A + zo * p.sAo + zi * p.sAi;
  const act_t* Wb = p.W + zo * p.sWo + zi * p.sWi;
  const int nsplit = p.ksplit > 1 ? p.ksplit : 1, sp = blockIdx.z;
  const long long coff = zo * p.sCo + zi * p.sCi + (nsplit > 1 ? (long long)sp * p.M * p.N : 0ll);
  const __amdgpu_buffer_rsrc_t rsA = __builtin_amdgcn_make_buffer_rsrc(const_cast<act_t*>(Ab), 0, OOB, 0x00020000);
  const __amdgpu_buffer_rsrc_t rsW = __builtin_amdgcn_make_buffer_rsrc(const_cast<act_t*>(Wb), 0, (unsigned)p.N * (unsigned)p.ldw * 2u, 0x00020000);

  int tapreg = 0;
#pragma unroll
  for (int j = 0; j < DMX_MAX_TAPS; ++j)
    if (lane == j) tapreg = (int)(unsigned char)p.tdy[j] | ((int)(unsigned char)p.tdx[j] << 8);

  const int lrow = lane >> 3, cc = (lane & 7) ^ lrow;
  const int cpt = p.Ci >> 3;
  const int HqWq = p.Hq * p.Wq;
  const unsigned lda2 = (unsigned)p.lda * 2u;
  unsigned a_lin[A_ISS], a_mask2[(A_ISS + 1) / 2];
  {
    int r_iy[A_ISS], r_ix[A_ISS];
    unsigned r_mask[A_ISS];
#pragma unroll
    for (int i = 0; i < A_ISS; ++i) {
      const int m = m0 + (i * NW + wave) * 8 + lrow;
      r_mask[i] = 0u; a_lin[i] = 0u;
      r_iy[i] = -(1 << 20); r_ix[i] = 0;
      if (m < mlim) {
        int b = 0, qy = 0, qx = m;
        if (!(p.Hq == 1 && p.Wq >= p.M)) {
          b = m / HqWq; const int rem = m - b * HqWq;
          qy = rem / p.Wq; qx = rem - qy * p.Wq;
        }
        r_iy[i] = qy * p.sy; r_ix[i] = qx * p.sx;
        a_lin[i] = (unsigned)b * (unsigned)(p.Hi * p.Wi) * lda2 + (unsigned)(r_iy[i] * p.Wi + r_ix[i]) * lda2 + ((unsigned)cc << 4);
      }
    }
    for (int t = 0; t < p.ntaps; ++t) {
      const int tv = __builtin_amdgcn_readlane(tapreg, t);
      const int dy = (int)(signed char)(tv & 0xff), dx = (int)(signed char)((tv >> 8) & 0xff);
#pragma unroll
      for (int i = 0; i < A_ISS; ++i)
        if ((unsigned)(r_iy[i] + dy) < (unsigned)p.Hi && (unsigned)(r_ix[i] + dx) < (unsigned)p.Wi) r_mask[i] |= 1u << t;
    }
#pragma unroll
    for (int i = 0; i < (A_ISS + 1) / 2; ++i) a_mask2[i] = 0u;
#pragma unroll
    for (int i = 0; i < A_ISS; ++i) a_mask2[i >> 1] |= r_mask[i] << ((i & 1) * 16);
  }
  const unsigned ldw2 = (unsigned)p.ldw * 2u;
  const unsigned w_row = (unsigned)(tn * BN + wave * 8 + lrow) * ldw2;
  const unsigned w_step = (unsigned)(NW * 8) * ldw2;

  const int kchunks = p.K >> 3;
// ... 158 lines not shown
          wait_step(ST);
          mfma_step(ST);
        });
      } else {
        static_for<0, NS>([&](auto ST) {
          constexpr int st = decltype(ST)::value;
          read_step(ST);
          wait_step(ST);
          mfma_step(ST);
          if constexpr (st < SPREAD) {
            static_for<st * PER / SPREAD, (st + 1) * PER / SPREAD>(issue_one);
            __builtin_amdgcn_sched_barrier(0);
          }
        });
      }
      asm volatile("s_waitcnt vmcnt(%0)\n\ts_waitcnt lgkmcnt(0)" ::"n"(KEEP) : "memory");
      __builtin_amdgcn_s_barrier();
      cur = cur + 1 == NSTAGE ? 0 : cur + 1;
      nxt = nxt + 1 == NSTAGE ? 0 : nxt + 1;
    }
    if constexpr (LAG) {
      __builtin_amdgcn_sched_barrier(0);
      if (nk > 0) static_for<LOWN, NS>(mfma_step);
    }
  };
  if constexpr (STAGGER) {
    if (wave >= NW / 2) kloop(std::true_type{}); else kloop(std::false_type{});
  } else {
    kloop(std::false_type{});
  }
#undef DMX_DSR
  asm volatile("s_waitcnt vmcnt(0)" ::: "memory");
  __builtin_amdgcn_s_barrier();
  DMX_GSTAMP(2);
  if constexpr (LNF) ln_apply<FM, FN, BN>(acc, s_ln, s_cs, wm * TM, wn * TN, lr, lq);
  if ((p.flags & EPI_F32OUT) || ((p.N | p.ldc | p.ldr | p.ldx | p.ldc2) & 7)) {
    gemm_epilogue<FM, FN>(p, acc, m0 + wm * TM, tn * BN + wn * TN, lr, lq, coff, HqWq);
  } else {
    constexpr int EPI_CH = EpiChunk<FM>::CH;
    constexpr int EPI_WAVE_BYTES = EPI_CH * (FN * 32 + 16) + EPI_CH * 12;
    static_assert(EPI_WAVE_BYTES * WM * WN <= 2 * (BM + BN) * 128, "epilogue staging does not fit the stage buffers");
    gemm_epilogue_lds<FM, FN, EM>(p, acc, m0 + wm * TM, tn * BN + wn * TN, lane, coff, HqWq, smem + wave * EPI_WAVE_BYTES, mlim);
  }
#ifdef DMX_GEMM_STAMPS
  DMX_GSTAMP(3);
  asm volatile("s_waitcnt vmcnt(0)" ::: "memory");
  DMX_GSTAMP(4);
  {
    const int wg = blockIdx.x + gridDim.x * (blockIdx.y + gridDim.y * blockIdx.z);
    if (tid == NW * 64 - 64 && wg < 8192) {
      unsigned hw, xcc;
      asm volatile("s_getreg_b32 %0, hwreg(HW_REG_HW_ID)" : "=s"(hw));
      asm volatile("s_getreg_b32 %0, hwreg(HW_REG_XCC_ID)" : "=s"(xcc));
#pragma unroll
      for (int i = 0; i < 5; ++i) g_gemm_stamps[wg * 6 + i] = gstamp_v[i];
      g_gemm_stamps[wg * 6 + 5] = ((unsigned long long)(xcc & 0xf) << 32) | hw;
    }
  }
#endif
}

__device__ __forceinline__ int xcd_remap(int bid) {
  const int nwg = gridDim.x, q = nwg >> 3, r = nwg & 7, xcd = bid & 7, loc = bid >> 3;
  return (xcd < r ? xcd * (q + 1) : r * (q + 1) + (xcd - r) * q) + loc;
}

template <int BM, int BN, int WM, int WN, int NSTAGE, int EM, bool LNF = false>
__global__ __launch_bounds__(WM* WN * 64) void gemm_glds_kernel(const GemmDesc p) {
  extern __shared__ __attribute__((aligned(16))) char smem[];
  const int tiles_n = (p.N + BN - 1) / BN;
  const int bid = xcd_remap(blockIdx.x);
  int m0 = (bid / tiles_n) * BM, mlim = p.M;
  if constexpr (EM == 5 || EM == 6) {
    const int P = p.Hq * p.Wq;
    if (P % (BM / WM) != 0) {
      const int tpi = (P + BM - 1) / BM, tm = bid / tiles_n, b = tm / tpi;
      m0 = b * P + (tm - b * tpi) * BM;
      mlim = (b + 1) * P;
    }
  }
  glds_tile<BM, BN, WM, WN, NSTAGE, EM, LNF>(p, smem, m0, bid % tiles_n, mlim);
}

template <int BM, int BN, int WM, int WN, int NSTAGE, int EM, bool LNF = false>
int launch_glds_t(const GemmDesc& d, hipStream_t stream) {
  constexpr int NT = WM * WN * 64;
  constexpr int SMEM = NSTAGE * (BM + BN) * 128 + (LNF ? BM * 8 + BN * 8 : 0);
  static_assert(SMEM <= 160 * 1024, "tile ring exceeds the 160 KiB of LDS");
  static bool attr_set = false;
  if (!attr_set) {
    hipFuncSetAttribute(reinterpret_cast<const void*>(&gemm_glds_kernel<BM, BN, WM, WN, NSTAGE, EM, LNF>),
                        hipFuncAttributeMaxDynamicSharedMemorySize, SMEM);
    attr_set = true;
  }
  long long tiles = (long long)cdiv(d.M, BM) * cdiv(d.N, BN);
  if constexpr (EM == 5 || EM == 6) {
    const int P = d.Hq * d.Wq;
    if (P % (BM / WM) != 0) tiles = (long long)(d.M / P) * cdiv(P, BM) * cdiv(d.N, BN);
  }
  dim3 grid((unsigned)tiles, (unsigned)d.Z, (unsigned)(d.ksplit > 1 ? d.ksplit : 1));
  static const bool bias_init = getenv("DMX_NO_BIAS_INIT") == nullptr;
  if (bias_init && (d.flags & EPI_BIAS) && d.bias && !(d.flags & (EPI_MASK | EPI_MASKBITS | EPI_SOFTBWD | EPI_LNFOLD))) {
    GemmDesc q = d;
    q.flags = (q.flags & ~EPI_BIAS) | EPI_BIASINIT;
    hipLaunchKernelGGL((gemm_glds_kernel<BM, BN, WM, WN, NSTAGE, EM, LNF>), grid, dim3(NT), SMEM, stream, q);
    return hipGetLastError() == hipSuccess ? DMX_OK : DMX_ERR_LAUNCH;
  }
  hipLaunchKernelGGL((gemm_glds_kernel<BM, BN, WM, WN, NSTAGE, EM, LNF>), grid, dim3(NT), SMEM, stream, d);
  return hipGetLastError() == hipSuccess ? DMX_OK : DMX_ERR_LAUNCH;
}
template <int BM, int BN, int WM, int WN, int EM, bool LNF = false>
int launch_cfg_t(const GemmDesc& d, hipStream_t stream) {
  constexpr int NT = WM * WN * 64;
  constexpr int SMEM = 2 * (BM + BN) * 128 + DMX_MAX_TAPS * 4 + (LNF ? BM * 8 + BN * 8 : 0);
  static bool attr_set = false;
  if (!attr_set) {
    hipFuncSetAttribute(reinterpret_cast<const void*>(&gemm_kernel<BM, BN, WM, WN, EM, LNF>),
                        hipFuncAttributeMaxDynamicSharedMemorySize, SMEM);
    attr_set = true;
  }
  long long tiles = (long long)cdiv(d.M, BM) * cdiv(d.N, BN);
  if constexpr (EM == 5 || EM == 6) {
    const int P = d.Hq * d.Wq;
    if (P % (BM / WM) != 0) tiles = (long long)(d.M / P) * cdiv(P, BM) * cdiv(d.N, BN);
  }
  dim3 grid((unsigned)tiles, (unsigned)d.Z, 1);
  static const bool bias_init = getenv("DMX_NO_BIAS_INIT") == nullptr;
  if (bias_init && (d.flags & EPI_BIAS) && d.bias && !(d.flags & (EPI_MASK | EPI_MASKBITS | EPI_SOFTBWD | EPI_LNFOLD))) {
    GemmDesc q = d;
    q.flags = (q.flags & ~EPI_BIAS) | EPI_BIASINIT;
    hipLaunchKernelGGL((gemm_kernel<BM, BN, WM, WN, EM, LNF>), grid, dim3(NT), SMEM, stream, q);
    return hipGetLastError() == hipSuccess ? DMX_OK : DMX_ERR_LAUNCH;
  }
  hipLaunchKernelGGL((gemm_kernel<BM, BN, WM, WN, EM, LNF>), grid, dim3(NT), SMEM, stream, d);
  return hipGetLastError() == hipSuccess ? DMX_OK : DMX_ERR_LAUNCH;
}
}
```

### diffmusic_amd/csrc/hifigan.hip

```cpp
#include "models.h"
#include "conv_pair.h"
#include <cstdlib>

struct SplitKScope {
  explicit SplitKScope(float* ws, size_t bytes, bool on) : on_(on && ws) { if (on_) dmx_gemm_set_splitk_workspace(ws, bytes); }
  ~SplitKScope() { if (on_) dmx_gemm_set_splitk_workspace(nullptr, 0); }
  bool on_;
};

struct Span { int a = 0, b = 0; bool empty() const { return b <= a; } };
static inline Span span_meet(Span x, Span y) { Span r{x.a > y.a ? x.a : y.a, x.b < y.b ? x.b : y.b}; if (r.empty()) r = Span{}; return r; }
static inline long long floor_div(long long a, long long b) { return a >= 0 ? a / b : -((-a + b - 1) / b); }
static inline long long ceil_div(long long a, long long b) { return -floor_div(-a, b); }

int dmx_conv_dead_rows_impl(int k, int dil, int pad, int stride, int transposed, int t_in, int t_out, int a, int b, int* lo, int* hi) {
  *lo = *hi = 0;
  if (k < 1 || dil < 1 || stride < 1 || pad < 0 || t_in < 1 || t_out < 1) return DMX_ERR_SHAPE;
  if (!transposed && stride != 1) return DMX_ERR_SHAPE;
  if (a < 0) a = 0;
  if (b > t_out) b = t_out;
  if (b <= a) return DMX_OK;
  const long long INF = 1ll << 40;
  const long long ea = a == 0 ? -INF : a, eb = b == t_out ? INF : b;
  long long l, h;
  if (!transposed) {
    l = ea - pad + (long long)(k - 1) * dil;
    h = eb - pad;
  } else {
    l = ceil_div(ea + pad, stride);
    h = ceil_div(eb - (k - 1) + pad, stride);
  }
  if (l < 0) l = 0;
  if (h > t_in) h = t_in;
  if (h > l) { *lo = (int)l; *hi = (int)h; }
  return DMX_OK;
}
static Span dead_in(const ConvLayer& L, Span d, int t_in, int t_out) {
  Span r;
  (void)dmx_conv_dead_rows_impl(L.kw, L.dil, L.pad_w, L.stride, L.transposed ? 1 : 0, t_in, t_out, d.a, d.b, &r.a, &r.b);
  return r;
}

struct DeadPlan {
  int B = 0, T = 0, s0 = 0, s1 = 0;
  bool on = false;
  Span wav;
  std::vector<Span> out, xs;
  std::vector<Span> xo, h, x;
  std::vector<int> skipped, total;
};

struct HifiGan : Model {
  dmx_hifigan_config cfg;
  DeadPlan plan;
  bool use_dead = false;
  static constexpr size_t kSplitKBytes = 32u << 20;
  float* splitk_ws = nullptr;
  ConvLayer conv_pre, conv_post;
  std::vector<ConvLayer> ups;
  std::vector<ConvLayer> c1, c2;
  int nk = 0, nd = 0, ns = 0;
  int B = 0, T = 0;
  std::vector<int> Ts;
  act_t* act_pre = nullptr;
  std::vector<act_t*> xs_a;
  std::vector<act_t*> ha, xa;
  std::vector<act_t*> act_out;
  std::vector<unsigned char*> hb, xb;
  std::vector<char> fused;
  float* wav8 = nullptr;
  bool have_tape = false;
  hipStream_t bstream[DMX_MAX_STAGES] = {};
  std::vector<hipEvent_t> events;
  size_t ev_next = 0;
  bool want_multi = true;
  hipEvent_t next_event() { hipEvent_t e = events[ev_next]; ev_next = (ev_next + 1) % events.size(); return e; }
  bool multi() const { return want_multi && !dry && !dmx_prof_is_active() && nk > 1; }
  bool multi_wanted() const { return want_multi && nk > 1; }

  int idx(int s, int k, int d) const { return (s * nk + k) * nd + d; }

  explicit HifiGan(const dmx_hifigan_config& c) : cfg(c) {
    kind = DMX_MODEL_HIFIGAN;
    ns = c.num_upsamples; nk = c.num_kernels; nd = c.num_dilations;
    const int C0 = c.upsample_initial_channel;
    conv_pre = make_conv1d(ps, "conv_pre", c.model_in_dim, C0, 7, 1, 3, true);
    for (int i = 0; i < ns; ++i) {
      const int s = c.upsample_rates[i], k = c.upsample_kernel_sizes[i];
      ups.push_back(make_convT1d(ps, "upsampler." + std::to_string(i), C0 >> i, C0 >> (i + 1), k, s, (k - s) / 2, true));
    }
    int ch = C0;
    for (int i = 0; i < ns; ++i) {
      ch = C0 >> (i + 1);
      for (int j = 0; j < nk; ++j) {
        const int k = c.resblock_kernel_sizes[j];
        const std::string pre = "resblocks." + std::to_string(i * nk + j);
        for (int d = 0; d < nd; ++d) {
          const int dil = c.resblock_dilation_sizes[j * nd + d];
          c1.push_back(make_conv1d(ps, pre + ".convs1." + std::to_string(d), ch, ch, k, dil, (k * dil - dil) / 2, true));
          c2.push_back(make_conv1d(ps, pre + ".convs2." + std::to_string(d), ch, ch, k, 1, (k - 1) / 2, true));
        }
      }
    }
    conv_post = make_conv1d(ps, "conv_post", ch, 1, 7, 1, 3, true);
    want_multi = getenv("DMX_MULTI_STREAM") != nullptr && getenv("DMX_SINGLE_STREAM") == nullptr;
    for (int k = 1; k < nk; ++k) (void)hipStreamCreateWithFlags(&bstream[k], hipStreamNonBlocking);
    events.resize(256);
    for (auto& e : events) (void)hipEventCreateWithFlags(&e, hipEventDisableTiming);
    splitk_ws = (float*)ps.dalloc(kSplitKBytes);
  }
  ~HifiGan() override {
    dmx_gemm_release_splitk_workspace(splitk_ws);
    for (int k = 1; k < nk; ++k) if (bstream[k]) (void)hipStreamDestroy(bstream[k]);
    for (auto& e : events) (void)hipEventDestroy(e);
  }

  int finalize(hipStream_t st) override {
    int rc = pack_layer(ps, conv_pre, st);
    for (auto& l : ups) if (rc == DMX_OK) rc = pack_layer(ps, l, st);
    for (auto& l : c1) if (rc == DMX_OK) rc = pack_layer(ps, l, st);
    for (auto& l : c2) if (rc == DMX_OK) rc = pack_layer(ps, l, st);
    if (rc == DMX_OK) rc = pack_layer(ps, conv_post, st);
    return rc;
  }

  bool step_is_fused(int id, int To) const {
    GemmDesc da, db;
    act_t* dummy = reinterpret_cast<act_t*>(size_t(256));
    unsigned char* dummyb = reinterpret_cast<unsigned char*>(size_t(256));
    Epi ea; ea.flags = EPI_LRELU2 | EPI_NO_C | EPI_BITS2; ea.act_slope = cfg.leaky_relu_slope; ea.B2 = dummyb;
    if (conv_fwd_1d_desc(c1[id], dummy, nullptr, B, To, ea, da) != DMX_OK) return false;
    Epi eb; eb.flags = EPI_RESID | EPI_RESID_INV | EPI_LRELU2 | EPI_NO_C | EPI_ACCUM; eb.R = dummy; eb.C2 = dummy;
    eb.resid_inv_slope = 1.f / cfg.leaky_relu_slope; eb.act_slope = cfg.leaky_relu_slope;
    if (conv_fwd_1d_desc(c2[id], nullptr, dummy, B, To, eb, db) != DMX_OK) return false;
    return dmx_conv_pair_eligible(&da, db);
  }

  void step_slabs(int id, int To, bool bwd, const PairDead& pd, int& skipped, int& total) const {
    GemmDesc da, db;
    act_t* dummy = reinterpret_cast<act_t*>(size_t(256));
    unsigned char* dummyb = reinterpret_cast<unsigned char*>(size_t(256));
    skipped = total = 0;
    if (!bwd) {
      Epi ea; ea.flags = EPI_LRELU2 | EPI_NO_C | EPI_BITS2; ea.act_slope = cfg.leaky_relu_slope; ea.B2 = dummyb;
      Epi eb; eb.flags = EPI_RESID | EPI_RESID_INV; eb.R = dummy; eb.resid_inv_slope = 1.f / cfg.leaky_relu_slope;
      if (conv_fwd_1d_desc(c1[id], dummy, nullptr, B, To, ea, da) != DMX_OK || conv_fwd_1d_desc(c2[id], nullptr, dummy, B, To, eb, db) != DMX_OK) return;
    } else {
      Epi ea; ea.flags = EPI_MASKBITS; ea.mask_slope = cfg.leaky_relu_slope; ea.XB = dummyb;
      Epi eb; eb.flags = EPI_RESID | EPI_MASKBITS; eb.mask_slope = cfg.leaky_relu_slope; eb.R = dummy; eb.XB = dummyb;
      if (conv_bwd_1d_desc(c2[id], dummy, dummy, B, To, ea, da) != DMX_OK || conv_bwd_1d_desc(c1[id], dummy, dummy, B, To, eb, db) != DMX_OK) return;
    }
    dmx_conv_pair_slabs(&da, db, &pd, &skipped, &total);
  }
// ... 133 lines not shown
          GemmDesc da[DMX_MAX_STAGES], db[DMX_MAX_STAGES];
          const GemmDesc* pa[DMX_MAX_STAGES]; const GemmDesc* pb[DMX_MAX_STAGES];
          PairDead pd[DMX_MAX_STAGES];
          for (int k = 0; k < nk; ++k) {
            const int id = idx(s, k, d);
            if (dead) pd[k] = dead_fwd(id);
            {
              Epi e; e.flags = EPI_LRELU2 | EPI_NO_C | EPI_BITS2; e.act_slope = slope; e.B2 = hb[id];
              RUN(conv_fwd_1d_desc(c1[id], xa[id], ha[id], B, To, e, da[k]));
            }
            if (d < nd - 1) {
              const int idn = idx(s, k, d + 1);
              act_t* xn = xa[idn];
              Epi e; e.flags = EPI_RESID | EPI_RESID_INV | EPI_LRELU2 | EPI_NO_C | EPI_BITS2; e.R = xa[id]; e.resid_inv_slope = 1.f / slope;
              e.act_slope = slope; e.C2 = xn; e.B2 = xb[idn];
              RUN(conv_fwd_1d_desc(c2[id], ha[id], xn, B, To, e, db[k]));
            } else {
              Epi e; e.flags = EPI_RESID | EPI_RESID_INV; e.R = xa[id]; e.resid_inv_slope = 1.f / slope; e.alpha = 1.f / nk;
              if (k > 0) e.flags |= EPI_ACCUM;
              if (k == nk - 1) { e.flags |= EPI_LRELU2 | EPI_NO_C; e.act_slope = next_slope; e.C2 = act_out[s]; }
              RUN(conv_fwd_1d_desc(c2[id], ha[id], sum, B, To, e, db[k]));
            }
            pa[k] = &da[k]; pb[k] = &db[k];
          }
          if (dry) continue;
          for (int k = 0; k < nk; ++k)
            if (!dmx_conv_pair_eligible(&da[k], db[k])) {
              dmx_set_error("hifigan: resblock step %d was planned as fused but the pair kernel refuses it", idx(s, k, d));
              return DMX_ERR_STATE;
            }
          if (d < nd - 1) RUN(dmx_conv_pair_group_launch(nk, pa, pb, st, dead ? pd : nullptr));
          else for (int k = 0; k < nk; ++k) RUN(conv_pair_run(da[k], db[k], st, dead ? &pd[k] : nullptr));
        }
        arena.release(mk);
        cur_act = act_out[s];
        Tin = To;
        continue;
      }
      hipEvent_t fin_prev = nullptr;
      if (mt) {
        hipEvent_t e0 = next_event();
        (void)hipEventRecord(e0, st);
        for (int k = 1; k < nk; ++k) (void)hipStreamWaitEvent(bstream[k], e0, 0);
      }
      for (int k = 0; k < nk; ++k) {
        hipStream_t sk = (mt && k > 0) ? bstream[k] : st;
        for (int d = 0; d < nd; ++d) {
          const int id = idx(s, k, d);
          const bool fz = fused[id] != 0;
          GemmDesc da, db;
          {
            Epi e; e.flags = EPI_LRELU2 | EPI_NO_C; e.act_slope = slope;
            if (fz) { e.flags |= EPI_BITS2; e.B2 = hb[id]; } else e.C2 = ha[id];
            RUN(conv_fwd_1d_desc(c1[id], xa[id], ha[id], B, To, e, da));
          }
          if (d < nd - 1) {
            const int idn = idx(s, k, d + 1);
            act_t* xn = xa[idn];
            Epi e; e.flags = EPI_RESID | EPI_RESID_INV | EPI_LRELU2 | EPI_NO_C; e.R = xa[id]; e.resid_inv_slope = 1.f / slope;
            e.act_slope = slope; e.C2 = xn;
            if (fused[idn]) { e.flags |= EPI_BITS2; e.B2 = xb[idn]; }
            RUN(conv_fwd_1d_desc(c2[id], ha[id], xn, B, To, e, db));
          } else {
            Epi e; e.flags = EPI_RESID | EPI_RESID_INV; e.R = xa[id]; e.resid_inv_slope = 1.f / slope; e.alpha = 1.f / nk;
            if (k > 0) e.flags |= EPI_ACCUM;
            if (k == nk - 1) { e.flags |= EPI_LRELU2 | EPI_NO_C; e.act_slope = next_slope; e.C2 = act_out[s]; }
            RUN(conv_fwd_1d_desc(c2[id], ha[id], sum, B, To, e, db));
          }
          if (!dry && fz && !dmx_conv_pair_eligible(&da, db)) {
            dmx_set_error("hifigan: resblock step %d was planned as fused but the pair kernel refuses it", id);
            return DMX_ERR_STATE;
          }
          if (d == nd - 1 && mt && fin_prev) (void)hipStreamWaitEvent(sk, fin_prev, 0);
          RUN(conv_pair_run(da, db, sk));
          if (d == nd - 1 && mt) { fin_prev = next_event(); (void)hipEventRecord(fin_prev, sk); }
        }
      }
      if (mt && fin_prev) (void)hipStreamWaitEvent(st, fin_prev, 0);
      arena.release(mk);
      cur_act = act_out[s];
      Tin = To;
    }
    const int Tout = Tin;
    wav8 = arena.f32((size_t)B * Tout * 8);
    CHECK_WS("hifigan");
    {
      Epi e; e.flags = EPI_F32OUT | EPI_TANH;
      RUN(conv_fwd_1d(conv_post, cur_act, wav8, B, Tout, e, st));
    }
    if (dead) RUN(dmx_gather_col_f32_dead(wav8, wav, (long long)B * Tout, 8, 0, Tout, plan.wav.a, plan.wav.b, st));
    else RUN(dmx_gather_col_f32(wav8, wav, (long long)B * Tout, 8, 0, st));
    have_tape = true;
    return DMX_OK;
  }

  int backward(const float* dwav, act_t* dmel, hipStream_t st) {
    if (!have_tape && !dry) { dmx_set_error("hifigan backward without forward"); return DMX_ERR_STATE; }
    SplitKScope sk_scope(splitk_ws, kSplitKBytes, !dry && !multi_wanted());
    const float slope = cfg.leaky_relu_slope;
    const int Tout = Ts[ns - 1];
    const size_t mk0 = arena.mark();
    act_t* gz = arena.bf((size_t)B * Tout * 8);
    const int Clast = ups[ns - 1].Cop;
    act_t* g = arena.bf((size_t)B * Tout * Clast);
    CHECK_WS("hifigan");
    const bool dead = use_dead && !dry;
    if (dead) RUN(dmx_tanh_bwd_pad8_dead(dwav, wav8, gz, (long long)B * Tout, Tout, plan.wav.a, plan.wav.b, st));
    else RUN(dmx_tanh_bwd_pad8(dwav, wav8, gz, (long long)B * Tout, st));
    {
      Epi e; e.flags = EPI_MASK; e.X = act_out[ns - 1]; e.mask_slope = 0.01f; e.alpha = 1.f / nk;
      RUN(conv_bwd_1d(conv_post, gz, g, B, Tout, e, st));
    }
    for (int s = ns - 1; s >= 0; --s) {
      const int To = Ts[s], Tin = s == 0 ? T : Ts[s - 1], C = ups[s].Cop;
      const size_t n = (size_t)B * To * C;
      act_t* gxs = arena.bf(n);
      act_t* ghk[DMX_MAX_STAGES];
      act_t* gAB[DMX_MAX_STAGES][2];
      for (int k = 0; k < nk; ++k) { ghk[k] = arena.bf(n); gAB[k][0] = arena.bf(n); gAB[k][1] = arena.bf(n); }
      const int Cin = ups[s].Cip;
      act_t* gprev = arena.bf((size_t)B * Tin * Cin);
      CHECK_WS("hifigan");
      const bool mt = multi();
      hipEvent_t fin_prev = nullptr;
      bool all_fused = nk <= 3;
      for (int k = 0; k < nk; ++k) for (int d = 0; d < nd; ++d) all_fused = all_fused && fused[idx(s, k, d)] != 0;
      if (all_fused && !mt) {
        const act_t* gcs[DMX_MAX_STAGES];
        for (int k = 0; k < nk; ++k) gcs[k] = g;
        if (dead && !plan.xs[s].empty() &&
            hipMemset2DAsync(gxs + (size_t)plan.xs[s].a * C, (size_t)To * C * sizeof(act_t), 0, (size_t)(plan.xs[s].b - plan.xs[s].a) * C * sizeof(act_t),
                             (size_t)B, st) != hipSuccess) {
          dmx_set_error("hifigan: clearing the dead rows of a stage gradient failed");
          return DMX_ERR_LAUNCH;
        }
        for (int d = nd - 1; d >= 0; --d) {
          GemmDesc da[DMX_MAX_STAGES], db[DMX_MAX_STAGES];
          const GemmDesc* pa[DMX_MAX_STAGES]; const GemmDesc* pb[DMX_MAX_STAGES];
          act_t* dsts[DMX_MAX_STAGES];
          PairDead pd[DMX_MAX_STAGES];
          for (int k = 0; k < nk; ++k) {
            const int id = idx(s, k, d);
            if (dead) pd[k] = dead_bwd(s, id, d);
            {
              Epi e; e.mask_slope = slope; e.flags = EPI_MASKBITS; e.XB = hb[id];
              RUN(conv_bwd_1d_desc(c2[id], gcs[k], ghk[k], B, To, e, da[k]));
            }
            Epi e; e.flags = EPI_RESID | EPI_MASKBITS; e.mask_slope = slope; e.R = gcs[k]; e.XB = xb[id];
            if (d == 0) { dsts[k] = gxs; if (k > 0) e.flags |= EPI_ACCUM; }
            else dsts[k] = (gcs[k] == gAB[k][0]) ? gAB[k][1] : gAB[k][0];
            RUN(conv_bwd_1d_desc(c1[id], ghk[k], dsts[k], B, To, e, db[k]));
            pa[k] = &da[k]; pb[k] = &db[k];
          }
          if (!dry) {
            if (d > 0) RUN(dmx_conv_pair_group_launch(nk, pa, pb, st, dead ? pd : nullptr));
            else for (int k = 0; k < nk; ++k) RUN(conv_pair_run(da[k], db[k], st, dead ? &pd[k] : nullptr));
          }
          for (int k = 0; k < nk; ++k) gcs[k] = dsts[k];
        }
      } else {
      if (mt) {
        hipEvent_t e0 = next_event();
        (void)hipEventRecord(e0, st);
        for (int k = 1; k < nk; ++k) (void)hipStreamWaitEvent(bstream[k], e0, 0);
      }
      for (int k = 0; k < nk; ++k) {
        hipStream_t sk = (mt && k > 0) ? bstream[k] : st;
        const act_t* gc = g;
        for (int d = nd - 1; d >= 0; --d) {
          const int id = idx(s, k, d);
          GemmDesc da, db;
          {
            Epi e; e.mask_slope = slope;
            if (fused[id]) { e.flags = EPI_MASKBITS; e.XB = hb[id]; } else { e.flags = EPI_MASK; e.X = ha[id]; }
            RUN(conv_bwd_1d_desc(c2[id], gc, ghk[k], B, To, e, da));
          }
          Epi e; e.flags = EPI_RESID; e.mask_slope = slope; e.R = gc;
          if (fused[id]) { e.flags |= EPI_MASKBITS; e.XB = xb[id]; } else { e.flags |= EPI_MASK; e.X = xa[id]; }
          act_t* dst;
          if (d == 0) {
            dst = gxs;
            if (k > 0) e.flags |= EPI_ACCUM;
            if (mt && fin_prev) (void)hipStreamWaitEvent(sk, fin_prev, 0);
          } else {
            dst = (gc == gAB[k][0]) ? gAB[k][1] : gAB[k][0];
          }
          RUN(conv_bwd_1d_desc(c1[id], ghk[k], dst, B, To, e, db));
          RUN(conv_pair_run(da, db, sk));
          if (d == 0 && mt) { fin_prev = next_event(); (void)hipEventRecord(fin_prev, sk); }
          gc = dst;
        }
      }
      }
      if (mt && fin_prev) (void)hipStreamWaitEvent(st, fin_prev, 0);
      {
        Epi e; e.flags = EPI_MASK; e.mask_slope = slope;
        if (s > 0) { e.X = act_out[s - 1]; e.alpha = 1.f / nk; } else { e.X = act_pre; }
        RUN(conv_bwd_1d(ups[s], gxs, gprev, B, Tin, e, st));
      }
      g = gprev;
    }
    {
      Epi e;
      RUN(conv_bwd_1d(conv_pre, g, dmel, B, T, e, st));
    }
    arena.release(mk0);
    return DMX_OK;
  }
};

Model* dmx_make_hifigan(const dmx_hifigan_config* c) { return new HifiGan(*c); }
int dmx_hifigan_out_len_impl(Model* m, int T) { return static_cast<HifiGan*>(m)->out_len(T); }
int dmx_hifigan_fwd_impl(Model* m, const act_t* mel, float* wav, int B, int T, void* ws, size_t wsb, hipStream_t st) {
  return static_cast<HifiGan*>(m)->forward(mel, wav, B, T, ws, wsb, st);
}
// ... 27 lines not shown
```

### diffmusic_amd/csrc/kernels.h

```cpp
#pragma once
#include "dmx_common.h"

#define DMX_GN_MAX_CHUNKS 512

size_t dmx_gn_scratch_floats(int B, int C, int G);
struct GnRegion {
  float* part = nullptr;
  int tm = 0, P = 0, nq = 0;
  int qoff = 0, cq = 0;
};
struct GnParts { int n = 0; GnRegion r[8]; };
size_t dmx_gn_part_floats(int B, int P, int N);
int dmx_groupnorm_fwd(const act_t* x, act_t* y, const float* gamma, const float* beta, float* stats, float* scale,
                      float* shift, float* partial, int B, int P, int C, int G, float eps, int silu, hipStream_t st,
                      const GnParts* parts = nullptr);
int dmx_groupnorm_bwd(const act_t* x, const act_t* dy, const act_t* add, act_t* dx, const float* stats,
                      const float* scale, const float* shift, float* k0, float* k1, float* partial, int B, int P, int C,
                      int G, int silu, hipStream_t st, const GnParts* parts = nullptr);
int dmx_layernorm_fwd(const act_t* x, act_t* y, const float* gamma, const float* beta, int rows, int C, float eps,
                      hipStream_t st);
int dmx_softmax_fwd(const float* S, act_t* P, const float* colbias, long long rows, int N, long long lds, long long ldp,
                    int rows_per_bias, hipStream_t st);
int dmx_softmax_act(const act_t* S, act_t* P, const float* colbias, long long rows, int N, long long ldp, int rows_per_bias,
                    hipStream_t st);
int dmx_rowdot(const act_t* a, const act_t* b, float* out, long long rows, int C, long long lda, long long ldb, hipStream_t st);
int dmx_geglu(const act_t* x, act_t* y, long long rows, int I, hipStream_t st);
int dmx_silu(const act_t* x, act_t* y, long long n, hipStream_t st);
int dmx_upsample_nearest(const act_t* x, act_t* y, int B, int Hi, int Wi, int Ho, int Wo, int C, hipStream_t st);
int dmx_upsample2x_bwd(const act_t* dy, act_t* dx, int B, int Hi, int Wi, int C, hipStream_t st);
int dmx_transpose(const act_t* in, act_t* out, int R, int C, long long ldi, long long ldo, int Z, int Zi, long long sIo,
                  long long sIi, long long sOo, long long sOi, hipStream_t st);
int dmx_concat2(const act_t* a, const act_t* b, act_t* dst, long long rows, int Ca, int Cb, hipStream_t st);
int dmx_copy_channels(const act_t* src, act_t* dst, long long rows, int C, int lds, int ldd, int soff, int doff,
                      hipStream_t st);
int dmx_axpby(const act_t* x, const act_t* y0, act_t* y, float a, float b, long long n, hipStream_t st);
int dmx_nchw_f32_to_nhwc_bf16(const float* x, act_t* y, int B, int C, int HW, int Cp, float scale, hipStream_t st);
int dmx_nhwc_bf16_to_nchw_f32(const act_t* x, float* y, int B, int C, int HW, int Cp, float scale, hipStream_t st);
int dmx_f32_to_bf16(const float* x, act_t* y, long long n, float scale, hipStream_t st);
int dmx_bf16_to_f32(const act_t* x, float* y, long long n, float scale, hipStream_t st);
int dmx_extract_col(const act_t* x, float* y, long long rows, int ld, int col, hipStream_t st);
int dmx_gather_col_f32(const float* x, float* y, long long rows, int ld, int col, hipStream_t st);
int dmx_tanh_bwd_pad8(const float* dwav, const float* wav8, act_t* gz, long long rows, hipStream_t st);
int dmx_gather_col_f32_dead(const float* x, float* y, long long rows, int ld, int col, int T, int s0, int s1, hipStream_t st);
int dmx_tanh_bwd_pad8_dead(const float* dwav, const float* wav8, act_t* gz, long long rows, int T, int s0, int s1, hipStream_t st);
int dmx_scatter_col_pad8(const float* v, act_t* y, long long rows, float scale, hipStream_t st);
int dmx_gather_col_f32_to_act(const float* x, act_t* y, long long rows, int ld, int col, hipStream_t st);
int dmx_pad_col8_act(const act_t* v, act_t* y, long long rows, hipStream_t st);
int dmx_timestep_embed(const float* t, act_t* y, int B, int dim, hipStream_t st);

bool dmx_flash_attn_ok(int dh, int C);
int dmx_flash_attn_fwd(const act_t* q, const act_t* k, const act_t* v, act_t* o, const float* colbias, int B, int Nq, int Nk,
                       int C, int heads, float scale, hipStream_t st, int ldq = 0, int ldk = 0, int ldv = 0, int* qt_out = nullptr);

int dmx_stft_tables(float* table, float* tableT, int n_fft, int bins, int Npad, int Kpad, int hann, hipStream_t st);
int dmx_stft_fwd(const float* wav, long long wav_stride, const float* table, float* X, int B, int L, int T, int n_fft, int hop, int Npad,
                 hipStream_t st);
int dmx_stft_bwd_frames(const float* Y, const float* tableT, float* dframe, int M, int n_fft, int Kpad, hipStream_t st);
int dmx_mel_fwd(const float* X, const float* fb, float* mel_lin, float* mel_out, int rows, int ldx, int bins, int n_mels, int power2,
                int to_db, float lo, float hi, hipStream_t st);
int dmx_mel_bwd(const float* X, const float* fb, const float* mel_lin, const float* dmel, float* Y, int rows, int ldx, int ldy, int bins,
                int n_mels, int power2, int to_db, float lo, float hi, hipStream_t st);
int dmx_stft_mag(const float* X, float* mag, int B, int T, int bins, int ldx, hipStream_t st);
int dmx_stft_mag_bwd(const float* X, const float* dmag, float* Y, int B, int T, int bins, int ldx, int ldy, hipStream_t st);
int dmx_overlap_add(const float* dframe, float* dwav, long long out_stride, int B, int T, int L, int n_fft, int hop, int accumulate,
                    hipStream_t st);
int dmx_l2_loss_grad(const float* ref, const float* pred, float* loss, float* dpred, int B, long long n, long long ref_stride, float gscale,
                     hipStream_t st);
int dmx_mask_mul(const float* x, long long xs, const float* mask, float* y, long long ys, int B, int L, int Ly, hipStream_t st);
int dmx_melscale(const float* mag, const float* fb, float* mel, int B, int T, int bins, int n_mels, float lo, float hi, hipStream_t st);
int dmx_absmax_normalize(float* x, float* inv_scale, int B, long long n, float target, hipStream_t st);

struct DmxStftMelTables {
  const float2* tw;
  const float* win;
  const int *klo, *klen; const float* fbc; int kmax;
  const int *mlo, *mlen; const float* fbr; int mmax;
};
int dmx_stft_mel_parts(int L, int hop);
int dmx_stft_mel_fwd(const DmxStftMelTables& t, const float* wav, long long wav_stride, const float* mask, const float* ref, long long ref_stride,
                     float* mel_out, float* partial, int B, int L, int hop, int power2, int to_db, float lo, float hi, hipStream_t st,
                     const float* add = nullptr, long long add_stride = 0, const float* addmag = nullptr, float nscale = 0.f,
                     const float* thr = nullptr);
int dmx_stft_mel_bwd(const DmxStftMelTables& t, const float* wav, long long wav_stride, const float* mask, const float* ref, long long ref_stride,
                     const float* dmel, const float* partial, float gscale, float* loss, float* dwav, long long dwav_stride, int Lfull,
                     int accumulate, int B, int L, int hop, int power2, int to_db, float lo, float hi, hipStream_t st,
                     const float* add = nullptr, long long add_stride = 0, const float* addmag = nullptr, float nscale = 0.f,
                     const float* thr = nullptr);

int dmx_tf_gain_frames(int L);
int dmx_tf_gain(const DmxStftMelTables& t, const float* x, long long x_stride, const float* gain, long long gain_clip_stride,
                long long gain_frame_stride, float* out, long long out_stride, int B, int L, int full, hipStream_t st);

int dmx_tf_wgrad_segments(int L);
int dmx_tf_wgrad(const DmxStftMelTables& t, const float* x, long long x_stride, const float* dy, long long dy_stride, float* part, int B, int L,
                 hipStream_t st);

constexpr int DMX_DRC_BLOCK = 64;

constexpr int DMX_DRC_FIT_SEGMENT = 256;
constexpr int DMX_DRC_FIT_PARAMS = 5;

constexpr int DMX_WARP_BLOCK = 64;


constexpr int DMX_CLICK_FRAME = 1024;
constexpr int DMX_CLICK_ORDER = 16;
constexpr int DMX_CLICK_MAX_GUARD = 64;

int dmx_pred_x0(const float* x, const float* eps, float* x0, long long n, float sqrt_a, float sqrt_1ma, hipStream_t st);
int dmx_pred_x0_ex(const float* x, const float* m, float* x0, long long n, float sqrt_a, float sqrt_1ma, int ptype, float clip_r, hipStream_t st);
int dmx_cfg_combine(const float* eps2, float* out, long long n, float scale, hipStream_t st);
int dmx_sched_update(int mode, const float* x, const float* eps, const float* x0, const float* g0, const float* inv_scale,
                     const float* noise, float* prev, float* x0_out, float* grad_out, int B, int n, float alpha_t, float alpha_prev,
                     float sigma, float rate, float eps_small, int global_norm, hipStream_t st, int ptype = 0, float clip_r = 0.f);
```

### diffmusic_amd/csrc/layers.hip

```cpp
#include "layers.h"
#include "conv_pair.h"
#include <cstdarg>

static thread_local char g_err[512] = "";
void dmx_set_error(const char* fmt, ...) {
  va_list ap;
  va_start(ap, fmt);
  vsnprintf(g_err, sizeof(g_err), fmt, ap);
  va_end(ap);
}
extern "C" const char* dmx_last_error() { return g_err; }

int ParamStore::add(const std::string& name, std::vector<int> shape) {
  Param p;
  p.name = name;
  p.shape = shape;
  p.numel = 1;
  for (int s : shape) p.numel *= (size_t)s;
  p.dev = (float*)dalloc(p.numel * sizeof(float));
  index[name] = (int)params.size();
  params.push_back(p);
  return (int)params.size() - 1;
}
void* ParamStore::dalloc(size_t bytes) {
  void* p = nullptr;
  if (hipMalloc(&p, bytes ? bytes : 16) != hipSuccess) { dmx_set_error("hipMalloc(%zu) failed", bytes); return nullptr; }
  owned.push_back(p);
  return p;
}
int ParamStore::load(const char* name, const float* host, size_t numel) {
  auto it = index.find(name);
  if (it == index.end()) { dmx_set_error("unknown parameter '%s'", name); return DMX_ERR_PARAM; }
  Param& p = params[it->second];
  if (p.numel != numel) { dmx_set_error("parameter '%s': expected %zu elements, got %zu", name, p.numel, numel); return DMX_ERR_PARAM; }
  if (hipMemcpy(p.dev, host, numel * sizeof(float), hipMemcpyHostToDevice) != hipSuccess) {
    dmx_set_error("hipMemcpy failed for '%s'", name);
    return DMX_ERR_PARAM;
  }
  p.loaded = true;
  return DMX_OK;
}
bool ParamStore::all_loaded(std::string* missing) const {
  for (const Param& p : params)
    if (!p.loaded) { if (missing) *missing = p.name; return false; }
  return true;
}
void ParamStore::free_all() {
  for (void* p : owned) (void)hipFree(p);
  owned.clear();
}

struct PackTaps { int idx[DMX_MAX_TAPS]; };
__host__ __device__ inline int geglu_src_row(int p, int half) {
  const int b = p >> 5, q = p & 31;
  return q < 16 ? 16 * b + q : half + 16 * b + (q - 16);
}
__global__ void pack_weight_kernel(const float* __restrict__ src, act_t* __restrict__ dst, int Np, int Nreal, int T, int Cp,
                                   int Creal, long long sn, long long sc, long long st, PackTaps taps, int geglu_half) {
  const long long idx = (long long)blockIdx.x * blockDim.x + threadIdx.x;
  const long long total = (long long)Np * T * Cp;
  if (idx >= total) return;
  const int c = (int)(idx % Cp);
  const int t = (int)((idx / Cp) % T);
  int n = (int)(idx / ((long long)Cp * T));
  if (geglu_half > 0) n = geglu_src_row(n, geglu_half);
  float v = 0.f;
  if (n < Nreal && c < Creal && taps.idx[t] >= 0) v = src[n * sn + c * sc + taps.idx[t] * st];
  dst[idx] = f2a(v);
}
__global__ void pad_bias_kernel(const float* __restrict__ src, float* __restrict__ dst, int n, int np, int geglu_half) {
  const int i = blockIdx.x * blockDim.x + threadIdx.x;
  const int s = geglu_half > 0 ? geglu_src_row(i, geglu_half) : i;
  if (i < np) dst[i] = (src && s < n) ? src[s] : 0.f;
}

__global__ __launch_bounds__(256) void ln_fold_kernel(const float* __restrict__ W, const float* __restrict__ gamma, const float* __restrict__ beta,
                                                      const float* __restrict__ bias, float* __restrict__ Wf, float* __restrict__ bf, int K) {
  __shared__ float sh[16];
  const int n = blockIdx.x;
  float acc = 0.f;
  for (int k = threadIdx.x; k < K; k += 256) {
    const float w = W[(long long)n * K + k];
    Wf[(long long)n * K + k] = w * gamma[k];
    acc += w * beta[k];
  }
// ... 185 lines not shown
  bool bias = false, bwd = false;
  for (int i = 0; i < n; ++i) {
    if (src[i]->Ci != Ci || src[i]->ntaps() != 1 || src[i]->transposed) { dmx_set_error("stacked projection: linear layers of equal input width"); return DMX_ERR_SHAPE; }
    Co += src[i]->Co; bias = bias || src[i]->has_bias; bwd = bwd || src[i]->need_bwd;
  }
  float *w = nullptr, *b = nullptr;
  if (hipMalloc(&w, (size_t)Co * Ci * sizeof(float)) != hipSuccess || hipMalloc(&b, (size_t)Co * sizeof(float)) != hipSuccess) {
    if (w) (void)hipFree(w);
    return DMX_ERR_PARAM;
  }
  (void)hipMemsetAsync(b, 0, (size_t)Co * sizeof(float), st);
  size_t off = 0;
  for (int i = 0; i < n; ++i) {
    (void)hipMemcpyAsync(w + off * Ci, ps.dev(src[i]->w_id), (size_t)src[i]->Co * Ci * sizeof(float), hipMemcpyDeviceToDevice, st);
    if (src[i]->has_bias) (void)hipMemcpyAsync(b + off, ps.dev(src[i]->b_id), (size_t)src[i]->Co * sizeof(float), hipMemcpyDeviceToDevice, st);
    off += src[i]->Co;
  }
  dst = ConvLayer();
  dst.Ci = Ci; dst.Co = Co; dst.Cip = pad8(Ci); dst.Cop = pad8(Co); dst.has_bias = bias; dst.need_bwd = bwd;
  const std::vector<int> all(1, 0);
  dst.wf.push_back(pack(ps, w, dst.Cop, Co, 1, dst.Cip, Ci, Ci, 1, 1, all, st));
  if (bwd) dst.wb = pack(ps, w, dst.Cip, Ci, 1, dst.Cop, Co, 1, Ci, 1, all, st);
  dst.bias = (float*)ps.dalloc(dst.Cop * sizeof(float));
  int rc = DMX_OK;
  if (!dst.wf[0] || (bwd && !dst.wb) || !dst.bias) rc = DMX_ERR_PARAM;
  else hipLaunchKernelGGL(pad_bias_kernel, dim3(cdiv(dst.Cop, 256)), dim3(256), 0, st, (const float*)b, dst.bias, Co, dst.Cop, 0);
  (void)hipStreamSynchronize(st);
  (void)hipFree(w); (void)hipFree(b);
  if (rc == DMX_OK && hipGetLastError() != hipSuccess) rc = DMX_ERR_LAUNCH;
  return rc;
}

static void init_desc(GemmDesc& d, const Epi& e) {
  memset(&d, 0, sizeof(d));
  d.Z = 1; d.Zi = 1;
  d.sy = d.sx = 1; d.osy = d.osx = 1;
  d.alpha = e.alpha; d.act_slope = e.act_slope; d.mask_slope = e.mask_slope; d.resid_inv_slope = e.resid_inv_slope;
  d.flags = e.flags;
  d.R = e.R; d.X = e.X; d.C2 = e.C2; d.rowbias = e.rowbias; d.ldrb = e.ldrb;
  d.XB = e.XB; d.B2 = e.B2;
  d.rowstats_out = e.rowstats_out; d.rowstats_in = e.rowstats_in; d.nslots = e.nslots;
  d.gn_part = e.gn_part;
  if (e.gn_part) d.flags |= e.gnb_x ? EPI_GNBWD : EPI_GNSTATS;
  d.gnb_x = e.gnb_x; d.gnb_scale = e.gnb_scale; d.gnb_shift = e.gnb_shift; d.gnb_silu = e.gnb_silu;
  d.gnb_stats = e.gnb_stats; d.gnb_cpg = e.gnb_cpg;
}
static void set_out(GemmDesc& d, void* C, int Ho, int Wo, int ldc) {
  d.C = C; d.Ho = Ho; d.Wo = Wo; d.ldc = d.ldr = d.ldx = d.ldc2 = ldc;
  d.ldxb = d.ldb2 = ldc >> 3;
  d.gnb_ldx = ldc;
}

int conv_out_len(const ConvLayer& L, int Ti) {
  if (L.transposed) return (Ti - 1) * L.stride - 2 * L.pad_w + L.kw;
  return (Ti + 2 * L.pad_w - L.dil * (L.kw - 1) - 1) / L.stride + 1;
}

static void fwd_1d_common(GemmDesc& d, const ConvLayer& L, const act_t* in, void* out, int Ti, int To, const Epi& e) {
  init_desc(d, e);
  if (L.has_bias) { d.bias = L.bias; d.flags |= EPI_BIAS; }
  d.A = in; d.Hi = 1; d.Wi = Ti; d.Ci = L.Cip; d.lda = L.Cip;
  d.N = L.Cop;
  set_out(d, out, 1, To, L.Cop);
}
int conv_fwd_1d_desc(const ConvLayer& L, const act_t* in, void* out, int B, int Ti, const Epi& e, GemmDesc& d) {
  if (L.transposed) return DMX_ERR_SHAPE;
  const int To = conv_out_len(L, Ti);
  fwd_1d_common(d, L, in, out, Ti, To, e);
  d.W = L.wf[0]; d.ntaps = L.kw; d.K = L.kw * L.Cip; d.ldw = d.K;
  d.Hq = 1; d.Wq = To; d.sx = L.stride; d.M = B * To;
  for (int t = 0; t < L.kw; ++t) { d.tdy[t] = 0; d.tdx[t] = (signed char)(t * L.dil - L.pad_w); }
  return DMX_OK;
}

int conv_fwd_1d(const ConvLayer& L, const act_t* in, void* out, int B, int Ti, const Epi& e, hipStream_t st) {
  const int To = conv_out_len(L, Ti);
  GemmDesc d;
  if (!L.transposed) {
    const int rc = conv_fwd_1d_desc(L, in, out, B, Ti, e, d);
    return rc != DMX_OK ? rc : dmx_gemm_launch(d, st);
  }
  fwd_1d_common(d, L, in, out, Ti, To, e);
  const int s = L.stride, p = L.pad_w;
  for (int r = 0; r < s; ++r) {
    GemmDesc q = d;
    const int nt = (int)L.wf_taps[r].size();
    const int base = (r + p) / s;
    q.W = L.wf[r]; q.ntaps = nt; q.K = nt * L.Cip; q.ldw = q.K;
    q.Hq = 1; q.Wq = cdiv(To - r, s); q.M = B * q.Wq;
    q.osx = s; q.oox = r;
    for (int i = 0; i < nt; ++i) { q.tdy[i] = 0; q.tdx[i] = (signed char)(base - i); }
    if (q.Wq <= 0) continue;
    const int rc = dmx_gemm_launch(q, st);
    if (rc != DMX_OK) return rc;
  }
  return DMX_OK;
}

int conv_bwd_1d_desc(const ConvLayer& L, const act_t* dout, void* din, int B, int Ti, const Epi& e, GemmDesc& d) {
  if (!L.wb) { dmx_set_error("layer has no dgrad weights"); return DMX_ERR_STATE; }
  const int To = conv_out_len(L, Ti);
  init_desc(d, e);
  d.A = dout; d.Hi = 1; d.Wi = To; d.Ci = L.Cop; d.lda = L.Cop;
  d.W = L.wb; d.ntaps = L.kw; d.K = L.kw * L.Cop; d.ldw = d.K;
  d.N = L.Cip;
  d.Hq = 1; d.Wq = Ti; d.M = B * Ti;
  set_out(d, din, 1, Ti, L.Cip);
  if (!L.transposed) {
    if (L.stride != 1) return DMX_ERR_SHAPE;
    for (int t = 0; t < L.kw; ++t) { d.tdy[t] = 0; d.tdx[t] = (signed char)(L.pad_w - t * L.dil); }
  } else {
    d.sx = L.stride;
    for (int t = 0; t < L.kw; ++t) { d.tdy[t] = 0; d.tdx[t] = (signed char)(t - L.pad_w); }
  }
  return DMX_OK;
}
int conv_bwd_1d(const ConvLayer& L, const act_t* dout, void* din, int B, int Ti, const Epi& e, hipStream_t st) {
  GemmDesc d;
  const int rc = conv_bwd_1d_desc(L, dout, din, B, Ti, e, d);
  return rc != DMX_OK ? rc : dmx_gemm_launch(d, st);
}

int conv_pair_run(const GemmDesc& a, const GemmDesc& b, hipStream_t st, const PairDead* dead) {
  if (dmx_conv_pair_eligible(&a, b)) return dmx_conv_pair_launch(&a, b, st, dead);
  if (dead) { dmx_set_error("conv_pair_run: dead rows need the fused pair kernel"); return DMX_ERR_SHAPE; }
  const int rc = dmx_gemm_launch(a, st);
  return rc != DMX_OK ? rc : dmx_gemm_launch(b, st);
}

int conv_fwd_2d(const ConvLayer& L, const act_t* in, void* out, int B, int Hi, int Wi, const Epi& e, hipStream_t st, int* gn_rows) {
  const int Ho = (Hi + L.pad_h + L.pad_h_hi - L.kh) / L.stride + 1, Wo = (Wi + L.pad_w + L.pad_w_hi - L.kw) / L.stride + 1;
  GemmDesc d;
  init_desc(d, e);
  if (L.has_bias) { d.bias = L.bias; d.flags |= EPI_BIAS; }
  d.A = in; d.Hi = Hi; d.Wi = Wi; d.Ci = L.Cip; d.lda = L.Cip;
  d.W = L.wf[0]; d.ntaps = L.kh * L.kw; d.K = d.ntaps * L.Cip; d.ldw = d.K;
  d.N = L.Cop; d.Hq = Ho; d.Wq = Wo; d.sy = d.sx = L.stride; d.M = B * Ho * Wo;
  set_out(d, out, Ho, Wo, L.Cop);
  for (int ky = 0; ky < L.kh; ++ky)
    for (int kx = 0; kx < L.kw; ++kx) {
      d.tdy[ky * L.kw + kx] = (signed char)(ky - L.pad_h);
      d.tdx[ky * L.kw + kx] = (signed char)(kx - L.pad_w);
    }
  return dmx_gemm_launch(d, st, gn_rows);
}

int conv_up2x_fwd(const ConvLayer& L, const act_t* in, void* out, int B, int Hi, int Wi, const Epi& e, hipStream_t st,
                  float* const* gn_buf, int* gn_rows) {
  if (L.wup.size() != 4) { dmx_set_error("layer has no upsample-folded weights"); return DMX_ERR_STATE; }
  for (int py = 0; py < 2; ++py)
    for (int px = 0; px < 2; ++px) {
      GemmDesc d;
      Epi ep = e;
      if (gn_buf) ep.gn_part = gn_buf[py * 2 + px];
      init_desc(d, ep);
      if (L.has_bias) { d.bias = L.bias; d.flags |= EPI_BIAS; }
      d.A = in; d.Hi = Hi; d.Wi = Wi; d.Ci = L.Cip; d.lda = L.Cip;
      d.W = L.wup[py * 2 + px]; d.ntaps = 4; d.K = 4 * L.Cip; d.ldw = d.K;
      d.N = L.Cop; d.Hq = Hi; d.Wq = Wi; d.M = B * Hi * Wi;
      set_out(d, out, 2 * Hi, 2 * Wi, L.Cop);
      d.osy = d.osx = 2; d.ooy = py; d.oox = px;
      for (int ty = 0; ty < 2; ++ty)
        for (int tx = 0; tx < 2; ++tx) {
          d.tdy[ty * 2 + tx] = (signed char)up2x_delta(py, ty);
          d.tdx[ty * 2 + tx] = (signed char)up2x_delta(px, tx);
        }
      const int rc = dmx_gemm_launch(d, st, gn_rows ? gn_rows + py * 2 + px : nullptr);
      if (rc != DMX_OK) return rc;
    }
  return DMX_OK;
}

int conv_up2x_bwd(const ConvLayer& L, const act_t* dout, void* din, int B, int Hi, int Wi, const Epi& e, hipStream_t st) {
  if (!L.wup_b) { dmx_set_error("layer has no upsample-folded dgrad weights"); return DMX_ERR_STATE; }
  GemmDesc d;
// ... 74 lines not shown
```

### include/diffmusic_hip.h

```cpp
#ifndef DIFFMUSIC_HIP_H
#define DIFFMUSIC_HIP_H
#include <stddef.h>
#include <stdint.h>

#ifdef __cplusplus
extern "C" {
#endif

#define DMX_ABI_VERSION 4
#define DMX_MAX_STAGES 8

typedef struct dmx_model dmx_model;

typedef struct dmx_hifigan_config {
  int model_in_dim;
  int upsample_initial_channel;
  int num_upsamples;
  int upsample_rates[DMX_MAX_STAGES];
  int upsample_kernel_sizes[DMX_MAX_STAGES];
  int num_kernels;
  int resblock_kernel_sizes[DMX_MAX_STAGES];
  int num_dilations;
  int resblock_dilation_sizes[DMX_MAX_STAGES * DMX_MAX_STAGES];
  float leaky_relu_slope;
// ... 138 lines not shown
int dmx_drc_pgrad(const float* state, const unsigned char* tape, const float* work, const float* bq0, const float* theta, float* part,
                  int batch, int L, float knee_db, void* stream);
int dmx_drc_update(const float* part, float* phi, float* m, float* v, float* theta, int batch, int L, int k, const double* lr, double beta1,
                   double beta2, double eps, float knee_db, const double* lo, const double* hi, void* stream);
int dmx_warp_fwd(const float* x, long long x_stride, const float* delay, long long delay_stride, float* y, int batch, int L, void* stream);
int dmx_warp_bwd(const float* dy, const float* delay, long long delay_stride, float* dx, int batch, int L, int full, void* stream);
int dmx_warp_wgrad(const float* dy, const float* x, long long x_stride, const float* delay, long long delay_stride, float* part, int batch,
                   int L, void* stream);
int dmx_warp_update(const float* part, float* coarse, float* m, float* v, float* fine, int batch, int L, int knot_stride, int k, double lr,
                    double beta1, double beta2, double eps, double max_delay, int anchor, void* stream);
int dmx_click_detect(const float* y, long long y_stride, float* a, float* e, float* sigma, unsigned char* flags, float* r, int batch, int L,
                     float threshold, float sigma_floor, void* stream);
int dmx_click_mask(const unsigned char* flags, float* mask, int* masked, int batch, int L, int guard, void* stream);
int dmx_mask_rows(const float* x, long long x_stride, const float* mask, long long mask_stride, float* y, int batch, int L, int Ly,
                  void* stream);
int dmx_declick_blend(const float* x, long long x_stride, const float* y, long long y_stride, const float* mask, long long mask_stride,
                      float* out, int batch, int L, int fade, void* stream);
int dmx_noise_add(const float* y, const float* z, float* out, long long n, float scale, void* stream);
int dmx_audio_stft_mag(dmx_audio* a, const float* wav, long long wav_stride, float* mag, void* state, int batch, int L, void* stream);
int dmx_audio_stft_mag_bwd(dmx_audio* a, const float* dmag, float* dwav, long long dwav_stride, void* state, int batch, int L,
                           int accumulate, void* stream);
int dmx_audio_tf_frames(int L);
int dmx_audio_tf_gain(dmx_audio* a, const float* x, long long x_stride, const float* gain, long long gain_clip_stride, float* out,
                      long long out_stride, int batch, int L, int full, void* stream);
int dmx_audio_tf_curve(dmx_audio* a, const float* x, long long x_stride, const float* curve, long long curve_clip_stride, float* out,
                       long long out_stride, int batch, int L, int full, void* stream);
int dmx_audio_tf_wgrad_segments(int L);
int dmx_audio_tf_wgrad(dmx_audio* a, const float* x, long long x_stride, const float* dy, long long dy_stride, float* partials, int batch, int L,
                       void* stream);
int dmx_audio_eq_update(const float* partials, int segments, float* g, float* m, float* v, int batch, int k, double lr, double beta1,
                        double beta2, double eps, int normalize, void* stream);
int dmx_audio_melscale(dmx_audio* a, const float* mag, float* mel_out, int batch, int frames, float lo, float hi, void* stream);
int dmx_mask_apply(const float* x, long long x_stride, const float* mask, float* y, long long y_stride, int batch, int L, int Ly,
                   void* stream);
int dmx_l2_loss(const float* ref, long long ref_stride, const float* pred, float* loss, float* dpred, int batch, long long n,
                float gscale, void* stream);
int dmx_track_stitch_fwd(const float* wav, long long wav_stride, float* track, const int* starts_host, int windows, int L, int R, int T,
                         void* stream);
int dmx_track_stitch_bwd(const float* dtrack, float* dwav, long long dwav_stride, const int* starts_host, int windows, int L, int R, int T,
                         int full, void* stream);
int dmx_stem_mix_fwd(const float* wav, long long wav_stride, float* mix, const float* gains_host, int stems, int groups, int L, void* stream);
int dmx_stem_mix_bwd(const float* dmix, float* dwav, long long dwav_stride, const float* gains_host, int stems, int groups, int L, int full,
                     void* stream);
int dmx_stem_project(const float* x, long long x_stride, const float* y, float* out, const float* gains_host, int stems, int L, void* stream);
int dmx_grad_normalize(float* x, float* inv_scale, int batch, long long n, float target, void* stream);

int dmx_fir_fwd(const float* in, long long in_stride, const float* h, float* out, long long out_stride, int batch, int Lin, int Lout,
                int taps, int orig, int new_, int off, void* stream);
int dmx_fir_bwd(const float* dout, long long dout_stride, const float* h, const float* h_rev, float* din, long long din_stride, int batch,
                int Lin, int Lout, int taps, int orig, int new_, int off, void* stream);
int dmx_fir_clip_fwd(const float* in, long long in_stride, const float* h, float* out, long long out_stride, int batch, int Lin, int Lout,
                     int taps, void* stream);
int dmx_fir_clip_bwd(const float* dout, long long dout_stride, const float* h, const float* h_rev, float* din, long long din_stride, int batch,
                     int Lin, int Lout, int taps, void* stream);
size_t dmx_fir_wgrad_workspace_floats(int batch, int Lout, int taps);
int dmx_fir_wgrad(const float* dy, long long dy_stride, const float* x, long long x_stride, float* partials, size_t partial_floats, int batch,
                  int L, int Lout, int taps, void* stream);
int dmx_ir_update(const float* partials, int segments, float* h, float* h_rev, float* m, float* v, int batch, int taps, double lr, double beta1,
                  double beta2, double eps, int k, void* stream);

#define DMX_SCHED_DDIM 0
#define DMX_SCHED_DPS 1
#define DMX_SCHED_MPGD 2
#define DMX_SCHED_DSG 3
#define DMX_SCHED_DIFFMUSIC 4
int dmx_sched_pred_x0(const float* x, const float* eps, float* x0, long long n, float alpha_t, void* stream);
int dmx_sched_pred_x0_ex(const float* x, const float* model_output, float* x0, long long n, float alpha_t, int prediction_type, float clip_range,
                         void* stream);
int dmx_sched_cfg_combine(const float* eps2, float* out, long long n, float scale, void* stream);
int dmx_sched_step(int mode, const float* x, const float* eps, const float* x0, const float* g0, const float* inv_scale,
                   const float* noise, float* prev, float* x0_out, float* grad_out, int batch, int n, float alpha_t, float alpha_prev,
                   float sigma, float rate, float eps_small, int global_norm, void* stream);
int dmx_sched_step_ex(int mode, const float* x, const float* eps, const float* x0, const float* g0, const float* inv_scale,
                      const float* noise, float* prev, float* x0_out, float* grad_out, int batch, int n, float alpha_t, float alpha_prev,
                      float sigma, float rate, float eps_small, int global_norm, int prediction_type, float clip_range, void* stream);

int dmx_randn_philox(float* out, int batch, long long n, const unsigned long long* seeds_host, unsigned long long offset, void* stream);

void dmx_prof_begin(void);
int dmx_prof_end(double* total_ms, double* total_flops);
int dmx_prof_dominant(double* ms, double* flops, double* bytes);

int dmx_gemm_raw(const void* desc, size_t desc_bytes, void* stream);
int dmx_flash_attn_raw(const void* q, const void* k, const void* v, void* o, const float* colbias, int B, int Nq, int Nk, int ldv,
                       int C, int heads, float scale, void* stream);
int dmx_flash_attn_ld_raw(const void* q, const void* k, const void* v, void* o, const float* colbias, int B, int Nq, int Nk, int ldq,
                          int ldk, int ldv, int C, int heads, float scale, int* qt_out, void* stream);
int dmx_softmax_raw(const float* S, void* P, const float* colbias, long long rows, int N, long long lds, long long ldp, int rows_per_bias,
                    void* stream);
int dmx_softmax_act_raw(const void* S, void* P, const float* colbias, long long rows, int N, long long ldp, int rows_per_bias, void* stream);
int dmx_transpose_raw(const void* in, void* out, int R, int C, long long ldi, long long ldo, int Z, int Zi, long long sIo, long long sIi,
                      long long sOo, long long sOi, void* stream);
int dmx_rowdot_raw(const void* a, const void* b, float* out, long long rows, int C, long long lda, long long ldb, void* stream);
int dmx_layernorm_raw(const void* x, void* y, const float* gamma, const float* beta, int rows, int C, float eps, void* stream);
int dmx_geglu_raw(const void* x, void* y, long long rows, int I, void* stream);
int dmx_gemm_splitk_workspace(void* ws, size_t bytes);
int dmx_conv_pair_raw(const void* desc_a, const void* desc_b, size_t desc_bytes, void* stream);
int dmx_conv_pair_dead_raw(const void* desc_a, const void* desc_b, size_t desc_bytes, const int* dead, int* skipped, int* total, void* stream);
int dmx_conv_pair_group_raw(int n, const void* descs_a, const void* descs_b, size_t desc_bytes, void* stream);
int dmx_conv_pair_group_dead_raw(int n, const void* descs_a, const void* descs_b, size_t desc_bytes, const int* dead, void* stream);
size_t dmx_groupnorm_scratch_floats(int B, int C, int G);
int dmx_groupnorm_raw(const void* x, void* y, const float* gamma, const float* beta, float* stats, float* scale, float* shift,
                      float* partial, int B, int P, int C, int G, float eps, int silu, void* stream);
size_t dmx_groupnorm_part_floats(int B, int P, int N);
int dmx_groupnorm_parts_raw(const void* x, void* y, const float* gamma, const float* beta, float* stats, float* scale, float* shift,
                            int B, int P, int C, int G, float eps, int silu, int nreg, float* const* part, const int* geom, void* stream);
int dmx_gemm_last_tile_rows_raw(void);
int dmx_conv2d_raw(const float* w_host, const float* b_host, const void* x, void* y, int B, int Hi, int Wi, int Ci, int Co, int k, int stride,
                   int pad_lo, int pad_hi, void* stream);
int dmx_groupnorm_bwd_raw(const void* x, const void* dy, const void* add, void* dx, const float* stats, const float* scale, const float* shift,
                          float* k0, float* k1, float* partial, int B, int P, int C, int G, int silu, int nreg, float* const* part,
                          const int* geom, void* stream);

#ifdef __cplusplus
}
#endif
#endif
```

Before: 27.19 steps/s (weak scaling: one step advances a batch of 8 clips on one GPU; value = K / wall x 1 GPU(s)).

## Add joint multi-phase transposed-conv GEMM launch and streaming HiFi-GAN conv_post kernels

```diff
diff --git a/diffmusic_amd/_lib.py b/diffmusic_amd/_lib.py
--- a/diffmusic_amd/_lib.py
+++ b/diffmusic_amd/_lib.py
@@ -107,6 +107,9 @@
     "dmx_gram_fwd": (C.c_int, [C.c_void_p, C.c_void_p, C.c_int, C.c_int, C.c_int, C.c_void_p]),
     "dmx_gram_bwd": (C.c_int, [C.c_void_p, C.c_void_p, C.c_void_p, C.c_int, C.c_int, C.c_int, C.c_void_p]),
     "dmx_gemm_raw": (C.c_int, [C.c_void_p, C.c_size_t, C.c_void_p]),
+    "dmx_gemm_phases_raw": (C.c_int, [C.c_int, C.c_void_p, C.c_size_t, C.c_void_p]),
+    "dmx_conv_post_fwd_raw": (C.c_int, [C.c_void_p] * 5 + [C.c_int] * 5 + [C.c_void_p]),
+    "dmx_conv_post_bwd_raw": (C.c_int, [C.c_void_p] * 5 + [C.c_int] * 3 + [C.c_float, C.c_float, C.c_int, C.c_int, C.c_void_p]),
     "dmx_prof_begin": (None, []),
     "dmx_prof_end": (C.c_int, [C.POINTER(C.c_double), C.POINTER(C.c_double)]),
     "dmx_flash_attn_raw": (C.c_int, [C.c_void_p, C.c_void_p, C.c_void_p, C.c_void_p, C.c_void_p] + [C.c_int] * 6 + [C.c_float, C.c_void_p]),
@@ -223,7 +226,8 @@
                "dmx_stem_mix_fwd", "dmx_stem_mix_bwd", "dmx_stem_project", "dmx_audio_tf_gain", "dmx_audio_tf_frames",
                "dmx_audio_tf_curve", "dmx_audio_tf_wgrad_segments", "dmx_audio_tf_wgrad", "dmx_audio_eq_update", "dmx_drc_fwd", "dmx_drc_bwd",
                "dmx_warp_fwd", "dmx_warp_bwd", "dmx_warp_wgrad", "dmx_warp_update", "dmx_drc_fwd_p", "dmx_drc_bwd_p", "dmx_drc_pgrad",
-               "dmx_drc_update", "dmx_click_detect", "dmx_click_mask", "dmx_mask_rows", "dmx_declick_blend")
+               "dmx_drc_update", "dmx_click_detect", "dmx_click_mask", "dmx_mask_rows", "dmx_declick_blend", "dmx_gemm_phases_raw",
+               "dmx_conv_post_fwd_raw", "dmx_conv_post_bwd_raw")
 
 _lib = None
 
@@ -232,7 +236,7 @@
     for name in ADDED_IN_V4:
         if not hasattr(h, name):
             raise RuntimeError(f"{path} reports ABI version {ABI_VERSION} but does not export `{name}` (a build from before the VAE "
-                               "encoder / track-mode / declipping / blind-dereverberation / source-separation / time-frequency-masking / blind-equalisation / de-compression / wow-and-flutter / blind-wow-and-flutter / blind-de-compression / declicking entry points): rebuild it (python -m diffmusic_amd.build --force)")
+                               "encoder / track-mode / declipping / blind-dereverberation / source-separation / time-frequency-masking / blind-equalisation / de-compression / wow-and-flutter / blind-wow-and-flutter / blind-de-compression / declicking / joint-phase-launch / streaming-conv_post entry points): rebuild it (python -m diffmusic_amd.build --force)")
 
 
 def lib():
diff --git a/diffmusic_amd/csrc/capi.hip b/diffmusic_amd/csrc/capi.hip
--- a/diffmusic_amd/csrc/capi.hip
+++ b/diffmusic_amd/csrc/capi.hip
@@ -187,6 +187,25 @@
   return dmx_gemm_launch(*reinterpret_cast<const GemmDesc*>(desc), ST(stream), &g_raw_gn_rows);
 }
 int dmx_gemm_last_tile_rows_raw(void) { return g_raw_gn_rows; }
+int dmx_gemm_phases_raw(int n, const void* descs, size_t desc_bytes, void* stream) {
+  if (desc_bytes != sizeof(GemmDesc)) { dmx_set_error("GemmDesc size mismatch: %zu vs %zu", desc_bytes, sizeof(GemmDesc)); return DMX_ERR_SHAPE; }
+  const int rc = dmx_gemm_launch_phases(reinterpret_cast<const GemmDesc*>(descs), n, ST(stream));
+  if (rc == DMX_ERR_SHAPE) dmx_set_error("descriptors not handled by the joint phase launch");
+  return rc;
+}
+
+int dmx_conv_post_fwd_raw(const void* x, const void* w, const float* bias, float* wav, float* keep, int B, int T, int C, int s0, int s1,
+                          void* stream) {
+  const int rc = dmx_conv_post_fwd((const act_t*)x, (const act_t*)w, bias, wav, keep, B, T, C, s0, s1, ST(stream));
+  if (rc == DMX_ERR_SHAPE) dmx_set_error("conv_post: B, T >= 1 and C a multiple of 8");
+  return rc;
+}
+int dmx_conv_post_bwd_raw(const float* dwav, const float* tw, const void* x, const void* w, void* g, int B, int T, int C, float slope,
+                          float alpha, int s0, int s1, void* stream) {
+  const int rc = dmx_conv_post_bwd(dwav, tw, (const act_t*)x, (const act_t*)w, (act_t*)g, B, T, C, slope, alpha, s0, s1, ST(stream));
+  if (rc == DMX_ERR_SHAPE) dmx_set_error("conv_post: B, T >= 1 and C a multiple of 8");
+  return rc;
+}
 
 int dmx_conv_pair_raw(const void* desc_a, const void* desc_b, size_t desc_bytes, void* stream) {
   if (desc_bytes != sizeof(GemmDesc)) { dmx_set_error("GemmDesc size mismatch: %zu vs %zu", desc_bytes, sizeof(GemmDesc)); return DMX_ERR_SHAPE; }
diff --git a/diffmusic_amd/csrc/conv_post.hip b/diffmusic_amd/csrc/conv_post.hip
--- /dev/null
+++ b/diffmusic_amd/csrc/conv_post.hip
@@ -0,0 +1,170 @@
+#include "kernels.h"
+
+namespace {
+constexpr int KW = 7, PAD = 3;
+constexpr int RO = 8;
+
+__device__ __forceinline__ void unpack8(const uint4 v, float (&f)[8]) {
+  f[0] = alo(v.x); f[1] = ahi(v.x); f[2] = alo(v.y); f[3] = ahi(v.y);
+  f[4] = alo(v.z); f[5] = ahi(v.z); f[6] = alo(v.w); f[7] = ahi(v.w);
+}
+
+template <int LPR, bool ONE>
+__global__ __launch_bounds__(256) void conv_post_fwd_kernel(const act_t* __restrict__ x, const act_t* __restrict__ w, const float* __restrict__ bias,
+                                                            float* __restrict__ wav, float* __restrict__ keep, int B, int T, int C, int s0, int s1) {
+  const long long gid = (long long)blockIdx.x * 256 + threadIdx.x;
+  const int sub = (int)(gid % LPR);
+  const long long grp = gid / LPR;
+  const int gpc = (T + RO - 1) / RO;
+  const long long b = grp / gpc;
+  if (b >= B) return;
+  const int t0 = (int)(grp - b * gpc) * RO;
+  const act_t* __restrict__ xb = x + b * (long long)T * C;
+  const int nch = ONE ? 1 : C / (8 * LPR);
+  float acc[RO];
+#pragma unroll
+  for (int o = 0; o < RO; ++o) acc[o] = sub == 0 ? bias[0] : 0.f;
+  float wr[KW][8];
+  if constexpr (ONE) {
+#pragma unroll
+    for (int j = 0; j < KW; ++j) unpack8(*reinterpret_cast<const uint4*>(w + j * C + sub * 8), wr[j]);
+  }
+  if (t0 >= s0 && (t0 + RO <= s1 || (s1 >= T && t0 < T))) {
+#pragma unroll
+    for (int o = 0; o < RO; ++o) {
+      const int t = t0 + o;
+      if ((o % LPR) != sub || t >= T) continue;
+      wav[b * T + t] = 0.f;
+      if (keep) keep[b * T + t] = 0.f;
+    }
+    return;
+  }
+#pragma unroll
+  for (int u = 0; u < RO + KW - 1; ++u) {
+    const int row = t0 + u - PAD;
+    const bool ok = row >= 0 && row < T;
+    for (int i = 0; i < nch; ++i) {
+      const int c = (sub + i * LPR) * 8;
+      float f[8];
+      unpack8(ok ? *reinterpret_cast<const uint4*>(xb + (long long)row * C + c) : make_uint4(0u, 0u, 0u, 0u), f);
+#pragma unroll
+      for (int o = 0; o < RO; ++o) {
+        const int j = u - o;
+        if (j < 0 || j >= KW) continue;
+        if constexpr (ONE) {
+#pragma unroll
+          for (int e = 0; e < 8; ++e) acc[o] = __builtin_fmaf(f[e], wr[j][e], acc[o]);
+        } else {
+          float wj[8];
+          unpack8(*reinterpret_cast<const uint4*>(w + j * C + c), wj);
+#pragma unroll
+          for (int e = 0; e < 8; ++e) acc[o] = __builtin_fmaf(f[e], wj[e], acc[o]);
+        }
+      }
+    }
+  }
+#pragma unroll
+  for (int o = 0; o < RO; ++o) {
+#pragma unroll
+    for (int m = 1; m < LPR; m <<= 1) acc[o] += __shfl_xor(acc[o], m, 64);
+  }
+#pragma unroll
+  for (int o = 0; o < RO; ++o) {
+    const int t = t0 + o;
+    if ((o % LPR) != sub || t >= T) continue;
+    const float v = (t >= s0 && t < s1) ? 0.f : tanhf(acc[o]);
+    wav[b * T + t] = v;
+    if (keep) keep[b * T + t] = v;
+  }
+}
+
+__global__ __launch_bounds__(256) void conv_post_bwd_kernel(const float* __restrict__ dwav, const float* __restrict__ tw, const act_t* __restrict__ x,
+                                                            const act_t* __restrict__ w, act_t* __restrict__ g, int B, int T, int C, float slope,
+                                                            float alpha, int s0, int s1) {
+  const long long gid = (long long)blockIdx.x * 256 + threadIdx.x;
+  const int cpr = C >> 3;
+  const int c = (int)(gid % cpr) * 8;
+  const long long grp = gid / cpr;
+  const int gpc = (T + RO - 1) / RO;
+  const long long b = grp / gpc;
+  if (b >= B) return;
+  const int u0 = (int)(grp - b * gpc) * RO;
+  float wr[KW][8];
+#pragma unroll
+  for (int j = 0; j < KW; ++j) unpack8(*reinterpret_cast<const uint4*>(w + j * C + c), wr[j]);
+  float gz[RO + KW - 1];
+#pragma unroll
+  for (int i = 0; i < RO + KW - 1; ++i) {
+    const int t = u0 - PAD + i;
+    float v = 0.f;
+    if (t >= 0 && t < T && !(t >= s0 && t < s1)) {
+      const float y = tw[b * T + t];
+      v = a2f(f2a(dwav[b * T + t] * (1.f - y * y)));
+    }
+    gz[i] = v;
+  }
+#pragma unroll
+  for (int o = 0; o < RO; ++o) {
+    const int u = u0 + o;
+    if (u >= T) break;
+    const long long off = (b * T + u) * (long long)C + c;
+    float xs[8], a[8];
+    unpack8(*reinterpret_cast<const uint4*>(x + off), xs);
+#pragma unroll
+    for (int e = 0; e < 8; ++e) a[e] = 0.f;
+#pragma unroll
+    for (int j = 0; j < KW; ++j) {
+#pragma unroll
+      for (int e = 0; e < 8; ++e) a[e] = __builtin_fmaf(gz[o + KW - 1 - j], wr[j][e], a[e]);
+    }
+#pragma unroll
+    for (int e = 0; e < 8; ++e) a[e] = (a[e] * (xs[e] > 0.f ? 1.f : slope)) * alpha;
+    *reinterpret_cast<uint4*>(g + off) = make_uint4(pack2a(a[0], a[1]), pack2a(a[2], a[3]), pack2a(a[4], a[5]), pack2a(a[6], a[7]));
+  }
+}
+
+__global__ __launch_bounds__(256) void zero_rows_kernel(act_t* __restrict__ x, long long per_clip, long long stride, long long first, long long total) {
+  const long long i = (long long)blockIdx.x * 256 + threadIdx.x;
+  if (i >= total) return;
+  const long long b = i / per_clip;
+  reinterpret_cast<uint4*>(x)[b * stride + first + (i - b * per_clip)] = make_uint4(0u, 0u, 0u, 0u);
+}
+
+template <int LPR, bool ONE>
+void fwd_launch(const act_t* x, const act_t* w, const float* bias, float* wav, float* keep, int B, int T, int C, int s0, int s1, hipStream_t st) {
+  const long long threads = (long long)B * ((T + RO - 1) / RO) * LPR;
+  hipLaunchKernelGGL((conv_post_fwd_kernel<LPR, ONE>), dim3((unsigned)((threads + 255) / 256)), dim3(256), 0, st, x, w, bias, wav, keep, B, T, C, s0, s1);
+}
+}
+
+bool dmx_conv_post_shape_ok(int B, int T, int C) {
+  return B >= 1 && T >= 1 && C >= 8 && (C & 7) == 0 && (long long)B * ((T + RO - 1) / RO) * (C >> 3) / 256 < (1ll << 31) - 1;
+}
+
+int dmx_conv_post_fwd(const act_t* x, const act_t* w, const float* bias, float* wav, float* keep, int B, int T, int C, int s0, int s1, hipStream_t st) {
+  if (!dmx_conv_post_shape_ok(B, T, C) || !x || !w || !bias || !wav) return DMX_ERR_SHAPE;
+  switch (C) {
+    case 8: fwd_launch<1, true>(x, w, bias, wav, keep, B, T, C, s0, s1, st); break;
+    case 16: fwd_launch<2, true>(x, w, bias, wav, keep, B, T, C, s0, s1, st); break;
+    case 32: fwd_launch<4, true>(x, w, bias, wav, keep, B, T, C, s0, s1, st); break;
+    case 64: fwd_launch<8, true>(x, w, bias, wav, keep, B, T, C, s0, s1, st); break;
+    default: fwd_launch<1, false>(x, w, bias, wav, keep, B, T, C, s0, s1, st); break;
+  }
+  return hipGetLastError() == hipSuccess ? DMX_OK : DMX_ERR_LAUNCH;
+}
+
+int dmx_conv_post_bwd(const float* dwav, const float* tw, const act_t* x, const act_t* w, act_t* g, int B, int T, int C, float slope, float alpha,
+                      int s0, int s1, hipStream_t st) {
+  if (!dmx_conv_post_shape_ok(B, T, C) || !dwav || !tw || !x || !w || !g) return DMX_ERR_SHAPE;
+  const long long threads = (long long)B * ((T + RO - 1) / RO) * (C >> 3);
+  hipLaunchKernelGGL(conv_post_bwd_kernel, dim3((unsigned)((threads + 255) / 256)), dim3(256), 0, st, dwav, tw, x, w, g, B, T, C, slope, alpha, s0, s1);
+  return hipGetLastError() == hipSuccess ? DMX_OK : DMX_ERR_LAUNCH;
+}
+
+int dmx_zero_rows(act_t* x, int B, int T, int C, int a, int b, hipStream_t st) {
+  if (!x || B < 1 || T < 1 || C < 8 || (C & 7) || a < 0 || b > T) return DMX_ERR_SHAPE;
+  if (b <= a) return DMX_OK;
+  const long long cpr = C >> 3, per_clip = (long long)(b - a) * cpr, total = per_clip * B;
+  hipLaunchKernelGGL(zero_rows_kernel, dim3((unsigned)((total + 255) / 256)), dim3(256), 0, st, x, per_clip, (long long)T * cpr, (long long)a * cpr, total);
+  return hipGetLastError() == hipSuccess ? DMX_OK : DMX_ERR_LAUNCH;
+}
diff --git a/diffmusic_amd/csrc/dmx_common.h b/diffmusic_amd/csrc/dmx_common.h
--- a/diffmusic_amd/csrc/dmx_common.h
+++ b/diffmusic_amd/csrc/dmx_common.h
@@ -139,6 +139,15 @@
   int gnb_cpg;
 };
 
+#define DMX_MAX_PHASES 8
+struct GemmPhases {
+  int n;
+  int ntaps[DMX_MAX_PHASES], Wq[DMX_MAX_PHASES], M[DMX_MAX_PHASES], oox[DMX_MAX_PHASES], dxs[DMX_MAX_PHASES];
+  const act_t* W[DMX_MAX_PHASES];
+};
+int dmx_gemm_launch_phases(const GemmDesc* q, int n, hipStream_t stream);
+int dmx_gemm_launch_phase_cfg(int cfg, const GemmDesc& d, const GemmPhases& ph, int mmax, hipStream_t stream);
+
 int dmx_gemm_launch(const GemmDesc& d, hipStream_t stream, int* gn_rows = nullptr);
 void dmx_gemm_set_splitk_workspace(float* ws, size_t bytes);
 void dmx_gemm_release_splitk_workspace(const float* ws);
diff --git a/diffmusic_amd/csrc/gemm_conv.hip b/diffmusic_amd/csrc/gemm_conv.hip
--- a/diffmusic_amd/csrc/gemm_conv.hip
+++ b/diffmusic_amd/csrc/gemm_conv.hip
@@ -286,14 +286,24 @@
   r.flops = flops; r.bytes = bytes; r.M = M; r.N = N; r.K = K; r.Z = 1; r.taps = taps; r.flags = flags; r.cfg = cfg;
 }
 
-int dmx_gemm_launch(const GemmDesc& d, hipStream_t stream, int* gn_rows) {
-  if (gn_rows) *gn_rows = 0;
+static int desc_checks(const GemmDesc& d) {
   if (d.M <= 0 || d.N <= 0 || d.K <= 0) return DMX_ERR_SHAPE;
   if ((d.Ci & 7) || (d.N & 3) || (d.K & 7) || (d.lda & 7) || (d.ldw & 7) || (d.ldc & 3)) return DMX_ERR_SHAPE;
   if (d.ntaps < 1 || d.ntaps > DMX_MAX_TAPS || d.K != d.ntaps * d.Ci) return DMX_ERR_SHAPE;
   if (d.Z < 1 || d.Zi < 1) return DMX_ERR_SHAPE;
   if ((d.flags & EPI_LRELU2) && !(d.act_slope >= 0.f && d.act_slope <= 1.f)) return DMX_ERR_SHAPE;
   if ((d.flags & EPI_RESID_INV) && !(d.resid_inv_slope >= 1.f)) return DMX_ERR_SHAPE;
+  if (d.flags & (EPI_MASKBITS | EPI_BITS2)) {
+    if ((d.flags & EPI_F32OUT) || ((d.N | d.ldc | d.ldr | d.ldx | d.ldc2) & 7) || d.Z != 1) return DMX_ERR_SHAPE;
+    if ((d.flags & EPI_MASKBITS) && (!d.XB || d.ldxb * 8 < d.N)) return DMX_ERR_SHAPE;
+    if ((d.flags & EPI_BITS2) && (!d.B2 || d.ldb2 * 8 < d.N)) return DMX_ERR_SHAPE;
+  }
+  return DMX_OK;
+}
+
+int dmx_gemm_launch(const GemmDesc& d, hipStream_t stream, int* gn_rows) {
+  if (gn_rows) *gn_rows = 0;
+  if (desc_checks(d) != DMX_OK) return DMX_ERR_SHAPE;
   if (d.flags & EPI_SOFTBWD) {
     if ((d.flags & ~(EPI_SOFTBWD)) || ((d.N | d.ldc | d.ldx) & 7) || !d.X || !d.rowbias || d.Zi != 1 || d.ntaps != 1) return DMX_ERR_SHAPE;
     if (!(d.osy == 1 && d.osx == 1 && d.ooy == 0 && d.oox == 0 && d.Ho == d.Hq && d.Wo == d.Wq)) return DMX_ERR_SHAPE;
@@ -302,11 +312,6 @@
     if ((d.flags & ~(EPI_GEGLU | EPI_BIAS | EPI_LNFOLD)) || (d.N & 31) || (d.ldc & 7) || d.ldc < d.N / 2 || d.alpha != 1.f) return DMX_ERR_SHAPE;
     if ((d.ldr | d.ldx | d.ldc2) & 7) return DMX_ERR_SHAPE;
     if (!(d.osy == 1 && d.osx == 1 && d.ooy == 0 && d.oox == 0 && d.Ho == d.Hq && d.Wo == d.Wq)) return DMX_ERR_SHAPE;
-  }
-  if (d.flags & (EPI_MASKBITS | EPI_BITS2)) {
-    if ((d.flags & EPI_F32OUT) || ((d.N | d.ldc | d.ldr | d.ldx | d.ldc2) & 7) || d.Z != 1) return DMX_ERR_SHAPE;
-    if ((d.flags & EPI_MASKBITS) && (!d.XB || d.ldxb * 8 < d.N)) return DMX_ERR_SHAPE;
-    if ((d.flags & EPI_BITS2) && (!d.B2 || d.ldb2 * 8 < d.N)) return DMX_ERR_SHAPE;
   }
   if ((d.flags & EPI_LNFOLD) && (d.flags & EPI_BIAS)) {
     GemmDesc q = d;
@@ -358,3 +363,89 @@
   g_prof_recs.push_back(r);
   return rc;
 }
+
+static double algo_bytes(const GemmDesc& d) {
+  const double mn = (double)d.M * d.N;
+  double by = 2.0 * d.N * (double)d.K;
+  if (!(d.flags & EPI_NO_C)) by += mn * ((d.flags & EPI_F32OUT) ? 4.0 : 2.0);
+  if (d.flags & EPI_ACCUM) by += mn * ((d.flags & EPI_F32OUT) ? 4.0 : 2.0);
+  if (d.flags & (EPI_RESID | EPI_RESID_INV)) by += mn * 2.0;
+  if (d.flags & EPI_MASK) by += mn * 2.0;
+  if (d.flags & EPI_MASKBITS) by += mn / 8.0;
+  if (d.flags & EPI_BITS2) by += mn / 8.0;
+  if (d.C2 && (d.flags & EPI_LRELU2)) by += mn * 2.0;
+  return by;
+}
+
+int dmx_gemm_launch_phases(const GemmDesc* q, int n, hipStream_t stream) {
+  if (!q || n < 2 || n > DMX_MAX_PHASES) return DMX_ERR_SHAPE;
+  int ref = 0, mmax = 0, kmin = q[0].K;
+  bool gl = true;
+  for (int r = 0; r < n; ++r) {
+    const GemmDesc& d = q[r];
+    if (desc_checks(d) != DMX_OK) return DMX_ERR_SHAPE;
+    if (d.flags & (EPI_SOFTBWD | EPI_GEGLU | EPI_LNFOLD | EPI_ROWSTATS | EPI_GNSTATS | EPI_GNBWD)) return DMX_ERR_SHAPE;
+    if (d.Z != 1 || d.Zi != 1 || d.ksplit > 1 || d.ldw != d.K || d.Hq < 1 || d.Wq < 1 || d.M % (d.Hq * d.Wq)) return DMX_ERR_SHAPE;
+    if (d.M / (d.Hq * d.Wq) != q[0].M / (q[0].Hq * q[0].Wq)) return DMX_ERR_SHAPE;
+    GemmDesc t = d;
+    t.W = q[0].W; t.ntaps = q[0].ntaps; t.K = q[0].K; t.ldw = q[0].ldw; t.Wq = q[0].Wq; t.M = q[0].M; t.oox = q[0].oox;
+    memcpy(t.tdy, q[0].tdy, sizeof(t.tdy)); memcpy(t.tdx, q[0].tdx, sizeof(t.tdx));
+    if (memcmp(&t, &q[0], sizeof(GemmDesc)) != 0) return DMX_ERR_SHAPE;
+    if (d.ntaps > q[ref].ntaps) ref = r;
+    if (d.M > mmax) mmax = d.M;
+    if (d.K < kmin) kmin = d.K;
+    gl = gl && glds_ok(d);
+  }
+  GemmDesc s = q[ref];
+  GemmPhases ph;
+  memset(&ph, 0, sizeof(ph));
+  ph.n = n;
+  double flops = 0.0, bytes = 2.0 * (double)(mmax / (s.Hq * s.Wq)) * s.Hi * s.Wi * s.Ci;
+  for (int r = 0; r < n; ++r) {
+    const GemmDesc& d = q[r];
+    const int dx = d.tdx[0] - s.tdx[0];
+    for (int i = 0; i < d.ntaps; ++i) {
+      if (d.tdy[i] != s.tdy[i] || d.tdx[i] != s.tdx[i] + dx) return DMX_ERR_SHAPE;
+    }
+    for (int i = 0; i < DMX_MAX_TAPS; ++i) if (s.tdx[i] + dx < -128 || s.tdx[i] + dx > 127) return DMX_ERR_SHAPE;
+    ph.W[r] = d.W; ph.ntaps[r] = d.ntaps; ph.Wq[r] = d.Wq; ph.M[r] = d.M; ph.oox[r] = d.oox; ph.dxs[r] = dx;
+    flops += 2.0 * d.M * (double)d.N * d.K;
+    bytes += algo_bytes(d);
+  }
+  int cfg = 0;
+  const long long nph = n;
+  if (s.tile_cfg) {
+    cfg = s.tile_cfg;
+  } else if (gl && mmax >= 2048 && s.N % 128 == 0) {
+    auto cost = [&](int bm, int bn, int slots, double eff) {
+      const double blocks = (double)cdiv(mmax, bm) * cdiv(s.N, bn) * nph;
+      return ceil(blocks / slots) * (bm / 128.0) * (bn / 128.0) * (slots / 256.0) / eff;
+    };
+    struct Cand { int cfg, bm, bn, slots; double eff; };
+    static const Cand cands[] = {{1, 256, 256, 256, 0.95}, {7, 320, 256, 256, 0.93}, {8, 192, 256, 256, 0.88}, {2, 256, 128, 256, 0.70},
+                                 {9, 320, 128, 256, 0.70}, {10, 192, 128, 256, 0.66}, {19, 512, 128, 256, 0.75}, {3, 128, 128, 512, 0.66}};
+    double bc = 1e30;
+    for (const Cand& c : cands) {
+      if (c.bn == 256 && s.N % 256) continue;
+      const double v = cost(c.bm, c.bn, c.slots, c.eff);
+      if (v < bc) { bc = v; cfg = c.cfg; }
+    }
+  } else if (s.N > 32 && (long long)cdiv(mmax, 128) * cdiv(s.N, 128) * nph < 200) {
+    cfg = gl && kmin >= 512 ? 12 : 6;
+  } else {
+    cfg = s.N > 64 ? 3 : (s.N > 32 ? 4 : 5);
+  }
+  const bool dma = !(cfg >= 3 && cfg <= 6);
+  if (dma && !gl) return DMX_ERR_SHAPE;
+  s.tile_cfg = 0;
+  if (!g_prof) return dmx_gemm_launch_phase_cfg(cfg, s, ph, mmax, stream);
+  ProfRec r;
+  (void)hipEventCreate(&r.a); (void)hipEventCreate(&r.b);
+  r.flops = flops; r.bytes = bytes;
+  r.M = mmax; r.N = s.N; r.K = s.K; r.Z = n; r.taps = s.ntaps; r.flags = s.flags; r.cfg = cfg;
+  (void)hipEventRecord(r.a, stream);
+  const int rc = dmx_gemm_launch_phase_cfg(cfg, s, ph, mmax, stream);
+  (void)hipEventRecord(r.b, stream);
+  g_prof_recs.push_back(r);
+  return rc;
+}
diff --git a/diffmusic_amd/csrc/gemm_phase.hip b/diffmusic_amd/csrc/gemm_phase.hip
--- /dev/null
+++ b/diffmusic_amd/csrc/gemm_phase.hip
@@ -0,0 +1,32 @@
+#include "gemm_tile.h"
+
+namespace {
+template <int BM, int BN, int WM, int WN, int NSTAGE>
+int ph_glds(const GemmDesc& d, const GemmPhases& ph, int mmax, hipStream_t stream) {
+  return (d.flags & (EPI_MASKBITS | EPI_BITS2)) ? launch_glds_phase_t<BM, BN, WM, WN, NSTAGE, 1>(d, ph, mmax, stream)
+                                                : launch_glds_phase_t<BM, BN, WM, WN, NSTAGE, 0>(d, ph, mmax, stream);
+}
+template <int BM, int BN, int WM, int WN>
+int ph_cfg(const GemmDesc& d, const GemmPhases& ph, int mmax, hipStream_t stream) {
+  return (d.flags & (EPI_MASKBITS | EPI_BITS2)) ? launch_cfg_phase_t<BM, BN, WM, WN, 1>(d, ph, mmax, stream)
+                                                : launch_cfg_phase_t<BM, BN, WM, WN, 0>(d, ph, mmax, stream);
+}
+}
+
+int dmx_gemm_launch_phase_cfg(int cfg, const GemmDesc& d, const GemmPhases& ph, int mmax, hipStream_t stream) {
+  switch (cfg) {
+    case 1: return ph_glds<256, 256, 2, 4, 2>(d, ph, mmax, stream);
+    case 2: return ph_glds<256, 128, 4, 2, 3>(d, ph, mmax, stream);
+    case 7: return ph_glds<320, 256, 2, 4, 2>(d, ph, mmax, stream);
+    case 8: return ph_glds<192, 256, 2, 4, 2>(d, ph, mmax, stream);
+    case 9: return ph_glds<320, 128, 4, 2, 2>(d, ph, mmax, stream);
+    case 10: return ph_glds<192, 128, 4, 2, 3>(d, ph, mmax, stream);
+    case 12: return ph_glds<64, 64, 2, 2, 4>(d, ph, mmax, stream);
+    case 19: return ph_glds<512, 128, 4, 2, 2>(d, ph, mmax, stream);
+    case 3: return ph_cfg<128, 128, 2, 2>(d, ph, mmax, stream);
+    case 4: return ph_cfg<128, 64, 2, 2>(d, ph, mmax, stream);
+    case 5: return ph_cfg<128, 32, 4, 1>(d, ph, mmax, stream);
+    case 6: return ph_cfg<64, 64, 2, 2>(d, ph, mmax, stream);
+    default: return DMX_ERR_SHAPE;
+  }
+}
diff --git a/diffmusic_amd/csrc/gemm_tile.h b/diffmusic_amd/csrc/gemm_tile.h
--- a/diffmusic_amd/csrc/gemm_tile.h
+++ b/diffmusic_amd/csrc/gemm_tile.h
@@ -60,8 +60,19 @@
   }
 }
 
+__device__ __forceinline__ GemmDesc phase_desc(const GemmDesc& p, const GemmPhases& ph, int r, int& dxs) {
+  GemmDesc q = p;
+  dxs = 0;
+#pragma unroll
+  for (int i = 0; i < DMX_MAX_PHASES; ++i)
+    if (r == i) { q.W = ph.W[i]; q.ntaps = ph.ntaps[i]; q.Wq = ph.Wq[i]; q.M = ph.M[i]; q.oox = ph.oox[i]; dxs = ph.dxs[i]; }
+  q.K = q.ntaps * p.Ci;
+  q.ldw = q.K;
+  return q;
+}
+
 template <int BM, int BN, int WM, int WN, int EM, bool LNF = false>
-__global__ __launch_bounds__(WM* WN * 64) void gemm_kernel(const GemmDesc p) {
+__device__ __forceinline__ void gemm_reg_tile(const GemmDesc& p, const GemmDesc& pt, const int dxs, char* smem, const int tm, const int tn) {
   constexpr int NT = WM * WN * 64;
   constexpr int TM = BM / WM, TN = BN / WN;
   constexpr int FM = TM / 16, FN = TN / 16;
@@ -70,19 +81,16 @@
   constexpr int A_BYTES = BM * 128, B_BYTES = BN * 128, STAGE = A_BYTES + B_BYTES;
   static_assert(A_PER >= 1 && B_PER >= 1, "tile too small for the thread count");
 
-  extern __shared__ __attribute__((aligned(16))) char smem[];
   short2* s_taps = reinterpret_cast<short2*>(smem + 2 * STAGE);
 
   const int tid = threadIdx.x;
-  const int tiles_n = (p.N + BN - 1) / BN;
-  const int tn = blockIdx.x % tiles_n, tm = blockIdx.x / tiles_n;
   const int z = blockIdx.y;
   const int zo = z / p.Zi, zi = z - zo * p.Zi;
   const act_t* __restrict__ Ab = p.A + zo * p.sAo + zi * p.sAi;
   const act_t* __restrict__ Wb = p.W + zo * p.sWo + zi * p.sWi;
   const long long coff = zo * p.sCo + zi * p.sCi;
 
-  if (tid < DMX_MAX_TAPS) s_taps[tid] = make_short2(p.tdy[tid], p.tdx[tid]);
+  if (tid < DMX_MAX_TAPS) s_taps[tid] = make_short2(pt.tdy[tid], (short)(pt.tdx[tid] + dxs));
   float2* s_ln = reinterpret_cast<float2*>(smem + 2 * STAGE + DMX_MAX_TAPS * 4);
   float* s_cs = reinterpret_cast<float*>(smem + 2 * STAGE + DMX_MAX_TAPS * 4 + BM * 8);
   int m0t = tm * BM, mlim = p.M;
@@ -221,6 +229,24 @@
     static_assert(EPI_WAVE_BYTES * WM * WN <= 2 * (BM + BN) * 128, "epilogue staging does not fit the stage buffers");
     gemm_epilogue_lds<FM, FN, EM>(p, acc, m0t + wm * TM, tn * BN + wn * TN, lane, coff, HqWq, smem + wave * EPI_WAVE_BYTES, mlim);
   }
+}
+
+template <int BM, int BN, int WM, int WN, int EM, bool LNF = false>
+__global__ __launch_bounds__(WM* WN * 64) void gemm_kernel(const GemmDesc p) {
+  extern __shared__ __attribute__((aligned(16))) char smem[];
+  const int tiles_n = (p.N + BN - 1) / BN;
+  gemm_reg_tile<BM, BN, WM, WN, EM, LNF>(p, p, 0, smem, blockIdx.x / tiles_n, blockIdx.x % tiles_n);
+}
+
+template <int BM, int BN, int WM, int WN, int EM>
+__global__ __launch_bounds__(WM* WN * 64) void gemm_phase_kernel(const GemmDesc p, const GemmPhases ph) {
+  extern __shared__ __attribute__((aligned(16))) char smem[];
+  const int tiles_n = (p.N + BN - 1) / BN;
+  const int t = blockIdx.x / tiles_n, tm = t / ph.n;
+  int dxs;
+  const GemmDesc q = phase_desc(p, ph, t - tm * ph.n, dxs);
+  if (tm * BM >= q.M) return;
+  gemm_reg_tile<BM, BN, WM, WN, EM, false>(q, p, dxs, smem, tm, blockIdx.x % tiles_n);
 }
 
 constexpr unsigned OOB = 0x80000000u;
@@ -545,6 +571,20 @@
   glds_tile<BM, BN, WM, WN, NSTAGE, EM, LNF>(p, smem, m0, bid % tiles_n, mlim);
 }
 
+template <int BM, int BN, int WM, int WN, int NSTAGE, int EM>
+__global__ __launch_bounds__(WM* WN * 64) void gemm_glds_phase_kernel(const GemmDesc p, const GemmPhases ph) {
+  extern __shared__ __attribute__((aligned(16))) char smem[];
+  const int tiles_n = (p.N + BN - 1) / BN;
+  const int bid = xcd_remap(blockIdx.x);
+  const int t = bid / tiles_n, tm = t / ph.n;
+  int dxs;
+  GemmDesc q = phase_desc(p, ph, t - tm * ph.n, dxs);
+#pragma unroll
+  for (int j = 0; j < DMX_MAX_TAPS; ++j) q.tdx[j] = (signed char)(p.tdx[j] + dxs);
+  if (tm * BM >= q.M) return;
+  glds_tile<BM, BN, WM, WN, NSTAGE, EM, false>(q, smem, tm * BM, bid % tiles_n, q.M);
+}
+
 template <int BM, int BN, int WM, int WN, int NSTAGE, int EM, bool LNF = false>
 int launch_glds_t(const GemmDesc& d, hipStream_t stream) {
   constexpr int NT = WM * WN * 64;
@@ -598,4 +638,40 @@
   hipLaunchKernelGGL((gemm_kernel<BM, BN, WM, WN, EM, LNF>), grid, dim3(NT), SMEM, stream, d);
   return hipGetLastError() == hipSuccess ? DMX_OK : DMX_ERR_LAUNCH;
 }
-}
+static inline bool phase_bias_init(const GemmDesc& d) {
+  static const bool bias_init = getenv("DMX_NO_BIAS_INIT") == nullptr;
+  return bias_init && (d.flags & EPI_BIAS) && d.bias && !(d.flags & (EPI_MASK | EPI_MASKBITS | EPI_SOFTBWD | EPI_LNFOLD));
+}
+template <int BM, int BN, int WM, int WN, int NSTAGE, int EM>
+int launch_glds_phase_t(const GemmDesc& d, const GemmPhases& ph, int mmax, hipStream_t stream) {
+  constexpr int NT = WM * WN * 64;
+  constexpr int SMEM = NSTAGE * (BM + BN) * 128;
+  static_assert(SMEM <= 160 * 1024, "tile ring exceeds the 160 KiB of LDS");
+  static bool attr_set = false;
+  if (!attr_set) {
+    hipFuncSetAttribute(reinterpret_cast<const void*>(&gemm_glds_phase_kernel<BM, BN, WM, WN, NSTAGE, EM>),
+                        hipFuncAttributeMaxDynamicSharedMemorySize, SMEM);
+    attr_set = true;
+  }
+  const long long tiles = (long long)cdiv(mmax, BM) * cdiv(d.N, BN) * ph.n;
+  GemmDesc q = d;
+  if (phase_bias_init(d)) q.flags = (q.flags & ~EPI_BIAS) | EPI_BIASINIT;
+  hipLaunchKernelGGL((gemm_glds_phase_kernel<BM, BN, WM, WN, NSTAGE, EM>), dim3((unsigned)tiles, 1, 1), dim3(NT), SMEM, stream, q, ph);
+  return hipGetLastError() == hipSuccess ? DMX_OK : DMX_ERR_LAUNCH;
+}
+template <int BM, int BN, int WM, int WN, int EM>
+int launch_cfg_phase_t(const GemmDesc& d, const GemmPhases& ph, int mmax, hipStream_t stream) {
+  constexpr int NT = WM * WN * 64;
+  constexpr int SMEM = 2 * (BM + BN) * 128 + DMX_MAX_TAPS * 4;
+  static bool attr_set = false;
+  if (!attr_set) {
+    hipFuncSetAttribute(reinterpret_cast<const void*>(&gemm_phase_kernel<BM, BN, WM, WN, EM>), hipFuncAttributeMaxDynamicSharedMemorySize, SMEM);
+    attr_set = true;
+  }
+  const long long tiles = (long long)cdiv(mmax, BM) * cdiv(d.N, BN) * ph.n;
+  GemmDesc q = d;
+  if (phase_bias_init(d)) q.flags = (q.flags & ~EPI_BIAS) | EPI_BIASINIT;
+  hipLaunchKernelGGL((gemm_phase_kernel<BM, BN, WM, WN, EM>), dim3((unsigned)tiles, 1, 1), dim3(NT), SMEM, stream, q, ph);
+  return hipGetLastError() == hipSuccess ? DMX_OK : DMX_ERR_LAUNCH;
+}
+}
diff --git a/diffmusic_amd/csrc/hifigan.hip b/diffmusic_amd/csrc/hifigan.hip
--- a/diffmusic_amd/csrc/hifigan.hip
+++ b/diffmusic_amd/csrc/hifigan.hip
@@ -69,6 +69,8 @@
   std::vector<unsigned char*> hb, xb;
   std::vector<char> fused;
   float* wav8 = nullptr;
+  float* wav_t = nullptr;
+  bool post_stream = false;
   bool have_tape = false;
   hipStream_t bstream[DMX_MAX_STAGES] = {};
   std::vector<hipEvent_t> events;
@@ -368,6 +370,16 @@
       Tin = To;
     }
     const int Tout = Tin;
+    static const bool want_stream = getenv("DMX_CONV_POST_GEMM") == nullptr;
+    post_stream = want_stream && conv_post.kw == 7 && conv_post.dil == 1 && conv_post.pad_w == 3 && conv_post.stride == 1 && conv_post.Co == 1 &&
+                  conv_post.has_bias && dmx_conv_post_shape_ok(B, Tout, conv_post.Cip);
+    if (post_stream) {
+      wav_t = arena.f32((size_t)B * Tout);
+      CHECK_WS("hifigan");
+      RUN(dmx_conv_post_fwd(cur_act, conv_post.wf[0], conv_post.bias, wav, wav_t, B, Tout, conv_post.Cip, dead ? plan.wav.a : 0, dead ? plan.wav.b : 0, st));
+      have_tape = true;
+      return DMX_OK;
+    }
     wav8 = arena.f32((size_t)B * Tout * 8);
     CHECK_WS("hifigan");
     {
@@ -386,14 +398,20 @@
     const float slope = cfg.leaky_relu_slope;
     const int Tout = Ts[ns - 1];
     const size_t mk0 = arena.mark();
-    act_t* gz = arena.bf((size_t)B * Tout * 8);
     const int Clast = ups[ns - 1].Cop;
-    act_t* g = arena.bf((size_t)B * Tout * Clast);
-    CHECK_WS("hifigan");
     const bool dead = use_dead && !dry;
-    if (dead) RUN(dmx_tanh_bwd_pad8_dead(dwav, wav8, gz, (long long)B * Tout, Tout, plan.wav.a, plan.wav.b, st));
-    else RUN(dmx_tanh_bwd_pad8(dwav, wav8, gz, (long long)B * Tout, st));
-    {
+    act_t* g;
+    if (post_stream) {
+      g = arena.bf((size_t)B * Tout * Clast);
+      CHECK_WS("hifigan");
+      RUN(dmx_conv_post_bwd(dwav, wav_t, act_out[ns - 1], conv_post.wf[0], g, B, Tout, Clast, 0.01f, 1.f / nk, dead ? plan.wav.a : 0,
+                            dead ? plan.wav.b : 0, st));
+    } else {
+      act_t* gz = arena.bf((size_t)B * Tout * 8);
+      g = arena.bf((size_t)B * Tout * Clast);
+      CHECK_WS("hifigan");
+      if (dead) RUN(dmx_tanh_bwd_pad8_dead(dwav, wav8, gz, (long long)B * Tout, Tout, plan.wav.a, plan.wav.b, st));
+      else RUN(dmx_tanh_bwd_pad8(dwav, wav8, gz, (long long)B * Tout, st));
       Epi e; e.flags = EPI_MASK; e.X = act_out[ns - 1]; e.mask_slope = 0.01f; e.alpha = 1.f / nk;
       RUN(conv_bwd_1d(conv_post, gz, g, B, Tout, e, st));
     }
@@ -414,9 +432,7 @@
       if (all_fused && !mt) {
         const act_t* gcs[DMX_MAX_STAGES];
         for (int k = 0; k < nk; ++k) gcs[k] = g;
-        if (dead && !plan.xs[s].empty() &&
-            hipMemset2DAsync(gxs + (size_t)plan.xs[s].a * C, (size_t)To * C * sizeof(act_t), 0, (size_t)(plan.xs[s].b - plan.xs[s].a) * C * sizeof(act_t),
-                             (size_t)B, st) != hipSuccess) {
+        if (dead && !plan.xs[s].empty() && dmx_zero_rows(gxs, B, To, C, plan.xs[s].a, plan.xs[s].b, st) != DMX_OK) {
           dmx_set_error("hifigan: clearing the dead rows of a stage gradient failed");
           return DMX_ERR_LAUNCH;
         }
diff --git a/diffmusic_amd/csrc/kernels.h b/diffmusic_amd/csrc/kernels.h
--- a/diffmusic_amd/csrc/kernels.h
+++ b/diffmusic_amd/csrc/kernels.h
@@ -45,6 +45,11 @@
 int dmx_tanh_bwd_pad8_dead(const float* dwav, const float* wav8, act_t* gz, long long rows, int T, int s0, int s1, hipStream_t st);
 int dmx_scatter_col_pad8(const float* v, act_t* y, long long rows, float scale, hipStream_t st);
 int dmx_gather_col_f32_to_act(const float* x, act_t* y, long long rows, int ld, int col, hipStream_t st);
+bool dmx_conv_post_shape_ok(int B, int T, int C);
+int dmx_conv_post_fwd(const act_t* x, const act_t* w, const float* bias, float* wav, float* keep, int B, int T, int C, int s0, int s1, hipStream_t st);
+int dmx_conv_post_bwd(const float* dwav, const float* tw, const act_t* x, const act_t* w, act_t* g, int B, int T, int C, float slope, float alpha,
+                      int s0, int s1, hipStream_t st);
+int dmx_zero_rows(act_t* x, int B, int T, int C, int a, int b, hipStream_t st);
 int dmx_pad_col8_act(const act_t* v, act_t* y, long long rows, hipStream_t st);
 int dmx_timestep_embed(const float* t, act_t* y, int B, int dim, hipStream_t st);
 
diff --git a/diffmusic_amd/csrc/layers.hip b/diffmusic_amd/csrc/layers.hip
--- a/diffmusic_amd/csrc/layers.hip
+++ b/diffmusic_amd/csrc/layers.hip
@@ -1,6 +1,7 @@
 #include "layers.h"
 #include "conv_pair.h"
 #include <cstdarg>
+#include <cstdlib>
 
 static thread_local char g_err[512] = "";
 void dmx_set_error(const char* fmt, ...) {
@@ -352,6 +353,7 @@
   }
   fwd_1d_common(d, L, in, out, Ti, To, e);
   const int s = L.stride, p = L.pad_w;
+  std::vector<GemmDesc> ph;
   for (int r = 0; r < s; ++r) {
     GemmDesc q = d;
     const int nt = (int)L.wf_taps[r].size();
@@ -361,6 +363,14 @@
     q.osx = s; q.oox = r;
     for (int i = 0; i < nt; ++i) { q.tdy[i] = 0; q.tdx[i] = (signed char)(base - i); }
     if (q.Wq <= 0) continue;
+    ph.push_back(q);
+  }
+  static const bool joint = getenv("DMX_NO_PHASE_JOINT") == nullptr;
+  if (joint && ph.size() > 1) {
+    const int rc = dmx_gemm_launch_phases(ph.data(), (int)ph.size(), st);
+    if (rc != DMX_ERR_SHAPE) return rc;
+  }
+  for (const GemmDesc& q : ph) {
     const int rc = dmx_gemm_launch(q, st);
     if (rc != DMX_OK) return rc;
   }
diff --git a/include/diffmusic_hip.h b/include/diffmusic_hip.h
--- a/include/diffmusic_hip.h
+++ b/include/diffmusic_hip.h
@@ -244,6 +244,11 @@
 int dmx_prof_dominant(double* ms, double* flops, double* bytes);
 
 int dmx_gemm_raw(const void* desc, size_t desc_bytes, void* stream);
+int dmx_gemm_phases_raw(int n, const void* descs, size_t desc_bytes, void* stream);
+int dmx_conv_post_fwd_raw(const void* x, const void* w, const float* bias, float* wav, float* keep, int B, int T, int C, int s0, int s1,
+                          void* stream);
+int dmx_conv_post_bwd_raw(const float* dwav, const float* tw, const void* x, const void* w, void* g, int B, int T, int C, float slope,
+                          float alpha, int s0, int s1, void* stream);
 int dmx_flash_attn_raw(const void* q, const void* k, const void* v, void* o, const float* colbias, int B, int Nq, int Nk, int ldv,
                        int C, int heads, float scale, void* stream);
 int dmx_flash_attn_ld_raw(const void* q, const void* k, const void* v, void* o, const float* colbias, int B, int Nq, int Nk, int ldq,
```

After: 27.45 steps/s (weak scaling: one step advances a batch of 8 clips on one GPU; value = K / wall x 1 GPU(s)) (median of 6 runs). Within noise of the previous version (+1.0%).
